# CESR-lab/mgroms

Measured on AMD Instinct MI355X. Metric: V-cycles/sec, seamount 512x512x64 (fine-grid smoother HBM GB/s and % of 8 TB/s: see roofline), higher is better.
Workload: dtype f64; 1 GPU; seamount 512x512x64 (1x1 ranks of 512x512x64), relax_method=FC, ns_pre=3 ns_post=2 ns_coarsest=40, cmatrix=real, interp=linear; levels=6, step=one Vcycle(1), nsmall=8

## Files before the change

### mgroms_amd/csrc/mgx_define.cpp

```cpp
#include "mgx_host.h"

namespace mgx_host {

int dmalloc(double **p, size_t n) {
  void *q = nullptr;
  HIPCHK(hipMalloc(&q, (n ? n : 1) * sizeof(double)));
  HIPCHK(hipMemsetAsync(q, 0, (n ? n : 1) * sizeof(double), S.stream));
  S.allocs.push_back(q);
  *p = (double *)q;
  return 0;
}

int roundup(int a, int m) { return (a + m - 1) / m * m; }

void make_view(LevView &v, int nx, int ny, int nz) {
  v.nx = nx; v.ny = ny; v.nz = nz;
  v.EO = 15;
  v.HO = roundup(16 + ny / 2, 16);
  v.RS = roundup(v.HO + ny / 2 + 1, 16);
  v.plane = (long long)nz * v.RS;
}

int find_grid_levels(int npxg, int npyg, int nx, int ny, int nz, int hold) {
  const int nxg = npxg * nx, nyg = npyg * ny, nzg = nz, ncoarsest = 4, nzmin = 2;
  const int nhoriz = nxg < nyg ? nxg : nyg;
  const int nl1 = 1 + (int)floor(log(nhoriz * 1.0 / ncoarsest * 1.0) / log(2.0));
  if (hold) {
    int l = 1;
    for (int z = nzg; l < nl1 && z != nzmin; l++) z = (z & 1) ? z : z / 2;
    return l;
  }
  const int nl2 = 1 + (int)floor(log(nzg * 1.0 / nzmin * 1.0) / log(2.0));
  return nl1 < nl2 ? nl1 : nl2;
}

void rank_level_table(int rank, std::vector<Level> &T, int npx0, int npy0, int nsmall, int periodic, int hold) {
  const int pi = rank % npx0, pj = rank / npx0;
  int nx = T[0].nx, ny = T[0].ny, nz = T[0].nz, npx = npx0, npy = npy0, incx = 1, incy = 1;
  T[0].npx = npx; T[0].npy = npy; T[0].incx = 1; T[0].incy = 1; T[0].gather = 0; T[0].ngx = 1; T[0].ngy = 1; T[0].key = 0; T[0].color = 0;
  for (int l = 1; l < (int)T.size(); l++) {
    Level &L = T[l];
    if (nz == 1 || (hold && (nz & 1))) { nx /= 2; ny /= 2; } else { nx /= 2; ny /= 2; nz /= 2; }
    L.gather = 0; L.ngx = 1; L.ngy = 1; L.key = 0; L.color = 0;
    if (((nx < ny ? nx : ny) < nsmall) && (npx * npy > 1)) {
      L.gather = 1;
      if (npx > 1) { npx /= 2; nx *= 2; L.ngx = 2; }
      if (npy > 1) { npy /= 2; ny *= 2; L.ngy = 2; }
      incx *= 2; incy *= 2;
    }
    L.nx = nx; L.ny = ny; L.nz = nz; L.npx = npx; L.npy = npy; L.incx = incx; L.incy = incy;
  }
  for (auto &L : T) {
    const int ix = L.incx, iy = L.incy;
    auto col = [&](int s) { const int t = pi + s * ix; return (t >= 0 && t < npx0) ? t : ((periodic & 1) ? ((t % npx0) + npx0) % npx0 : -1); };
    auto row = [&](int s) { const int t = pj + s * iy; return (t >= 0 && t < npy0) ? t : ((periodic & 2) ? ((t % npy0) + npy0) % npy0 : -1); };
    static const int di[8] = {0, 1, 0, -1, -1, 1, 1, -1}, dj[8] = {-1, 0, 1, 0, -1, -1, 1, 1};
    for (int d = 0; d < 8; d++) {
      const int c = col(di[d]), r = row(dj[d]);
      L.neighb[d] = (c >= 0 && r >= 0) ? r * npx0 + c : -1;
    }
  }
  for (int l = 1; l < (int)T.size(); l++) {
    Level &L = T[l];
    if (!L.gather) continue;
    const int ix = L.incx / 2, iy = L.incy / 2;
    const int family = (pi / ix) * ix * iy + npx0 * iy * (pj / iy);
    const int nextfamily = (pi / (2 * ix)) * ix * iy * 4 + npx0 * 2 * iy * (pj / (iy * 2));
    L.color = nextfamily + (pi % ix) + (pj % iy) * ix;
    const int N = ix * npx0;
    L.key = ((family % N) / (ix * iy)) % 2 + 2 * ((family / N) % 2);
  }
}

int gather2d(Level &L, double *src_tmp, double *dst) {
  const int nxc = L.nx / L.ngx, nyc = L.ny / L.ngy, Ng = nxc * nyc;
  rect(src_tmp, L.blk, 3, 1, 1, nyc, 1, nyc, 1, nxc);
  if (!S.ag) return fail("a gather is needed but mgx_set_comm was not called");
  if (S.ag(S.ctx, L.group, L.ngroup, L.blk, L.gbuf, Ng)) return fail("allgather callback failed");
  for (int q = 0; q < L.ngroup; q++) {
    const int l = q % L.ngx, m = q / L.ngx;
    rect(dst, L.gbuf + (size_t)q * Ng, 4, 1, 1, L.ny, 1 + m * nyc, (m + 1) * nyc, 1 + l * nxc, (l + 1) * nxc);
  }
  return 0;
}

void set_window_planes(bool known) {
  for (int l = 0; l < S.nlevs && l < 32; l++) {
    Level &L = S.lev[l];
    if (!L.v.gk || !S.rho_dev || !known) { L.rbs_rho = -1.0; L.rbs_m = 0; L.rbs_rows = L.nz; continue; }
    L.rbs_rho = S.rho_host[l];
    L.rbs_m = mgxk_rbseq_window_planes(L.rbs_rho);
    L.rbs_rows = (L.gdec && !L.gdec_h.empty()) ? mgxk_rbseq_window_rows(L.gdec_h.data(), L.nz) : L.nz;
    if (S.verbose > 1 && S.rank == 0) printf(" level %d: red-black walk contracts by %.4g per plane: %d planes of warm-up%s\n", l + 1, L.rbs_rho, L.rbs_m, L.rbs_m ? "" : " (none: the walk over the whole level stays)");
  }
}

static bool zeta_chain() {
  for (int l = 0; l < S.nlevs; l++) {
    const Level &L = S.lev[l];
    if (L.gather || !all_physical(sides_of(L))) return false;
    if (l > 0 && (2 * L.nx != S.lev[l - 1].nx || 2 * L.ny != S.lev[l - 1].ny)) return false;
  }
  const int D = mgxs_zeta_chain_depth();
  for (int s = 0;; s += D) {
    const int nd = std::min(D, S.nlevs - 1 - s);
    double *a[16];
    for (int d = 0; d <= nd; d++) a[d] = S.lev[s + d].g.zeta;
    mgxs_zeta_chain(S.stream, a, S.lev[s].ny, S.lev[s].nx, nd); S.n_launch++;
    if (s + nd >= S.nlevs - 1) break;
  }
  return true;
}

static int wrap_rmask(Level &L) {
  for (int ax = 0; ax < 2; ax++) {
    if (!(S.periodic & (1 << ax))) continue;
    const int lo = ax == 0 ? 3 : 0, hi = ax == 0 ? 1 : 2;
    const bool first = ax == 0 ? S.pi == 0 : S.pj == 0, last = ax == 0 ? S.pi == S.npx - 1 : S.pj == S.npy - 1;
    const int nn = ax == 0 ? L.nx : L.ny, cnt = (ax == 0 ? L.ny : L.nx) + 2;
    if ((size_t)cnt > S.xbuf_n) return fail("halo buffer too small");
    auto line = [&](double *buf, int op, int c) { if (ax == 0) rect(L.g.rmask, buf, op, 1, 1, L.ny, 0, L.ny + 1, c, c); else rect(L.g.rmask, buf, op, 1, 1, L.ny, c, c, 0, L.nx + 1); };
    int n = 0, peer[2], cn[2], dr[2]; double *sb[2], *rb[2];
    if (first) { line(S.xbuf[lo], 3, 1); peer[n] = L.neighb[lo]; cn[n] = cnt; sb[n] = S.xbuf[lo]; rb[n] = S.xbuf[8 + lo]; dr[n] = lo; n++; }
    if (last) { line(S.xbuf[hi], 3, nn); peer[n] = L.neighb[hi]; cn[n] = cnt; sb[n] = S.xbuf[hi]; rb[n] = S.xbuf[8 + hi]; dr[n] = hi; n++; }
    if (!n) continue;
    CHK(exchange(n, peer, sb, rb, cn, dr));
    if (first) line(S.xbuf[8 + lo], 4, 0);
    if (last) line(S.xbuf[8 + hi], 4, nn + 1);
  }
  return 0;
}

int define_matrices(int what, bool may_return_early) {
  const bool all = what == DM_ALL;
  const bool wait = !(may_return_early && S.async_ops) || (S.rho_dev && S.rb_seq);
  if (S.rho_dev) HIPCHK(hipMemsetAsync(S.rho_dev, 0, sizeof S.rho_host, S.stream));
  const bool chained = !all && zeta_chain();
  if (chained) S.n_zeta_chain++;
  for (int l = 0; l < S.nlevs; l++) {
    Level &L = S.lev[l];
    if (l > 0) {
      Level &F = S.lev[l - 1];
      const int nxc = L.gather ? L.nx / L.ngx : L.nx, nyc = L.gather ? L.ny / L.ngy : L.ny;
      double *src[4] = {F.g.dx, F.g.dy, F.g.zeta, F.g.h};
      double *own[4] = {L.g.dx, L.g.dy, L.g.zeta, L.g.h};
      const double fac[4] = {0.5, 0.5, 0.25, 0.25};
      for (int q = 0; q < 4; q++) {
        if (!all && (q != 2 || chained)) continue;
        mgxs_coarsen2d(S.stream, src[q], L.gather ? L.tmp2[q] : own[q], F.ny, nyc, nxc, fac[q]); S.n_launch++;
        if (L.gather) CHK(gather2d(L, L.tmp2[q], own[q]));
      }
    }
    if (all) CHK(rl_fill_halo(L, L.g.dx, 1, 1, 0));
    if (all) CHK(rl_fill_halo(L, L.g.dy, 1, 1, 0));
    if (!chained) CHK(rl_fill_halo(L, L.g.zeta, 1, 1, 0));
    if (all) CHK(rl_fill_halo(L, L.g.h, 1, 1, 0));
    if (all && l == 0 && S.par.bmask && S.periodic) CHK(wrap_rmask(L));
    mgxs_zr_zw(S.stream, &L.g, S.hlim, S.theta_b, S.theta_s); S.n_launch++;
    CHK(rl_fill_halo(L, L.g.zr, L.nz, 2, 0));
    CHK(rl_fill_halo(L, L.g.zw, L.nz + 1, 2, 0));
    L.g.bmask = S.par.bmask ? 1 : 0;
    if (l > 0 && all) {
      rect(L.g.rmask, 0, 5, 1, 1, L.ny, 0, L.ny + 1, 0, L.nx + 1);
      if (S.par.bmask) {
        if (L.neighb[0] < 0) rect(L.g.rmask, 0, 2, 1, 1, L.ny, 0, 0, 0, L.nx + 1);
        if (L.neighb[1] < 0) rect(L.g.rmask, 0, 2, 1, 1, L.ny, 0, L.ny + 1, L.nx + 1, L.nx + 1);
        if (L.neighb[2] < 0) rect(L.g.rmask, 0, 2, 1, 1, L.ny, L.ny + 1, L.ny + 1, 0, L.nx + 1);
        if (L.neighb[3] < 0) rect(L.g.rmask, 0, 2, 1, 1, L.ny, 0, L.ny + 1, 0, 0);
      }
    }
    L.g.szx = L.g.szy + (size_t)L.nz * (L.ny + 2) * (L.nx + 2);
    mgxs_slopes_ref(S.stream, &L.g); S.n_launch++;
    mgxs_define_matrix(S.stream, &L.g, l == 0, 0); S.n_launch += 2;
    if (S.par.bmask) for (int s = 0; s < 8; s++) CHK(rl_fill_halo(L, L.g.cA + (size_t)s * L.nz * (L.ny + 2) * (L.nx + 2), L.nz, 1, 0, true));
    mgxs_define_matrix(S.stream, &L.g, l == 0, 1); S.n_launch++;
    if (l == 0) {
      mgxm_ref2model(S.stream, L.g.zw, L.g.mzw, L.nz + 1, 2, L.nx, L.ny);
      mgxm_ref2model(S.stream, L.g.dzw, L.g.mdzw, L.nz + 1, 1, L.nx, L.ny);
      mgxm_ref2model(S.stream, L.g.cw, L.g.mcw, L.nz + 1, 1, L.nx, L.ny);
      mgxm_ref2model(S.stream, L.g.zxdy, L.g.mzxdy, L.nz, 1, L.nx, L.ny);
      mgxm_ref2model(S.stream, L.g.zydx, L.g.mzydx, L.nz, 1, L.nx, L.ny);
      S.n_launch += 5;
      if (all) {
        mgxm_ref2model_2d(S.stream, L.g.dx, L.g.mdx, L.nx, L.ny);
        mgxm_ref2model_2d(S.stream, L.g.dy, L.g.mdy, L.nx, L.ny);
        mgxm_ref2model_2d(S.stream, L.g.rmask, L.g.mrmask, L.nx, L.ny);
        S.n_launch += 3;
      }
    }
    if (L.nz <= 1024) { mgxk_convert8(S.stream, &L.v, L.g.cA); S.n_launch++; }
    else for (int s = 0; s < 8; s++) { mgxk_convert(S.stream, &L.v, L.v.cA[s], L.g.cA + (size_t)s * L.nz * (L.ny + 2) * (L.nx + 2), 1, 0, 0); S.n_launch++; }
    mgxs_pivots(S.stream, &L.v); S.n_launch++;
    if (L.v.gk) { mgxk_rbseq_setup(S.stream, &L.v); S.n_launch++; }
    if (L.v.gk && S.rho_dev && l < 32) { mgxk_rbseq_rho(S.stream, &L.v, S.rho_dev + l); S.n_launch++; }
    if (L.v.gk && L.gdec) {
      HIPCHK(hipMemsetAsync(L.gdec, 0, (size_t)L.nz * sizeof(double), S.stream));
      mgxk_rbseq_gdecay(S.stream, &L.v, L.gdec); S.n_launch++;
      if (wait) HIPCHK(hipMemcpyAsync(L.gdec_h.data(), L.gdec, (size_t)L.nz * sizeof(double), hipMemcpyDeviceToHost, S.stream));
    }
    L.v.zy = L.zy_store; L.v.zx = L.zx_store;
    if (L.nz <= 1024) { mgxk_convert2(S.stream, &L.v, L.zy_store, L.zx_store, L.g.szy); S.n_launch++; }
    else { mgxk_convert(S.stream, &L.v, L.zy_store, L.g.szy, 1, 0, 0); mgxk_convert(S.stream, &L.v, L.zx_store, L.g.szx, 1, 0, 0); S.n_launch += 2; }
    L.v.m4 = L.f2d_store[0]; L.v.d4 = L.f2d_store[1]; L.v.m7 = L.f2d_store[2]; L.v.d7 = L.f2d_store[3];
    L.v.h2 = L.f2d_store[4]; L.v.hi2 = L.f2d_store[5]; L.v.ze2 = L.f2d_store[6]; L.v.cffw = L.tab_store[0]; L.v.csw = L.tab_store[1];
    L.v.dx2 = L.zg_store[0]; L.v.dy2 = L.zg_store[1]; L.v.cffr = L.zg_store[2]; L.v.csr = L.zg_store[3];
    if (all) { mgxs_zw_js(S.stream, &L.g, &L.v, S.hlim, S.theta_b, S.theta_s); S.n_launch += 3; }
    else { mgxs_ze2_js(S.stream, &L.g, &L.v); S.n_launch++; }
    if (S.no_mf || S.par.bmask) { L.v.zy = L.v.zx = nullptr; L.v.m4 = nullptr; }
  }
  if (wait) {
    if (S.rho_dev) HIPCHK(hipMemcpyAsync(S.rho_host, S.rho_dev, sizeof S.rho_host, hipMemcpyDeviceToHost, S.stream));
    CHK(sync_stream());
  }
  set_window_planes(wait);
  S.cd_valid = 0;
  S.coef_gen++;
  S.have_matrix = true;
  S.have_geometry = true;
  return 0;
}

ModelView model_view() {
  double *m = S.call_mask ? S.d_rmask_m : (S.par.bmask ? S.lev[0].g.mrmask : nullptr);
  return ModelView{S.d_u, S.d_v, S.d_w, m, S.par.bmask ? 1 : 0};
}

int set_call_mask(const double *rmask, bool dev) {
  S.call_mask = rmask != nullptr;
  if (!rmask) return 0;
  Level &L = S.lev[0];
  const size_t n2 = (size_t)(L.ny + 2) * (L.nx + 2) * sizeof(double);
  HIPCHK(hipMemcpyAsync(S.d_rmask_ref, rmask, n2, dev ? hipMemcpyDeviceToDevice : hipMemcpyHostToDevice, S.stream));
  mgxm_ref2model_2d(S.stream, S.d_rmask_ref, S.d_rmask_m, L.nx, L.ny); S.n_launch++;
  return 0;
}

int flux_halo(Level &L, int face, double *fx) {
  const int lo = face == 0 ? L.neighb[3] : L.neighb[0], hi = face == 0 ? L.neighb[1] : L.neighb[2];
  const int last = face == 0 ? L.nx + 1 : L.ny + 1, cnt = L.nz * (face == 0 ? L.ny : L.nx);
  if (lo < 0) { mgxm_flux_zero_face(S.stream, &L.g, fx, face, 1); S.n_launch++; }
  if (hi < 0) { mgxm_flux_zero_face(S.stream, &L.g, fx, face, last); S.n_launch++; }
  if (lo < 0 && hi < 0) return 0;
  if ((size_t)cnt > S.xbuf_n) return fail("halo buffer too small");
  int n = 0, peer[2], cn[2], dr[2]; double *sb[2], *rb[2];
  if (lo >= 0) { mgxm_flux_face_copy(S.stream, &L.g, fx, S.xbuf[0], face, 1, 0); S.n_launch++; peer[n] = lo; cn[n] = cnt; sb[n] = S.xbuf[0]; rb[n] = S.xbuf[8]; dr[n] = face == 0 ? 3 : 0; n++; }
  if (hi >= 0) { peer[n] = hi; cn[n] = cnt; sb[n] = S.xbuf[2]; rb[n] = S.xbuf[9]; dr[n] = face == 0 ? 1 : 2; n++; }
  if (hi >= 0) HIPCHK(hipMemsetAsync(S.xbuf[2], 0, (size_t)cnt * sizeof(double), S.stream));
  CHK(exchange(n, peer, sb, rb, cn, dr));
  if (hi >= 0) { mgxm_flux_face_copy(S.stream, &L.g, fx, S.xbuf[9], face, last, 1); S.n_launch++; }
  return 0;
}

int compute_rhs_dev() {
  Level &L = S.lev[0];
  TicScope ts(1, "compute_rhs");
  ModelView M = model_view();
  HIPCHK(hipMemsetAsync(L.v.b, 0, L.n3js * sizeof(double), S.stream));
  mgxm_rhs_uf(S.stream, &L.g, &M, S.d_fx); S.n_launch++;
  if (!S.par.bmask) CHK(flux_halo(L, 0, S.d_fx));
  mgxm_rhs_vf(S.stream, &L.g, &M, S.d_fy); S.n_launch++;
  if (!S.par.bmask) CHK(flux_halo(L, 1, S.d_fy));
  mgxm_rhs_wf(S.stream, &L.g, &M, S.d_fz); S.n_launch++;
  mgxm_rhs_accum(S.stream, &L.g, S.d_bm, S.d_fx, S.d_fy, S.d_fz); S.n_launch++;
  mgxm_js_model(S.stream, &L.v, L.v.b, S.d_bm, 1); S.n_launch++;
  return 0;
}

int correct_uvw_dev() {
  Level &L = S.lev[0];
  TicScope ts(1, "correct_uvw");
  ModelView M = model_view();
  mgxm_js_model(S.stream, &L.v, L.v.p, S.d_bm, 0); S.n_launch++;
  mgxm_correct_uvw(S.stream, &L.g, S.d_bm, &M); S.n_launch++;
  return 0;
}

int upload_uvw(const double *u, const double *v, const double *w) {
  Level &L = S.lev[0];
  const size_t nu = (size_t)(L.nx + 1) * (L.ny + 2) * L.nz, nv = (size_t)(L.nx + 2) * (L.ny + 1) * L.nz, nw = (size_t)(L.nx + 2) * (L.ny + 2) * (L.nz + 1);
  HIPCHK(hipMemcpyAsync(S.d_u, u, nu * sizeof(double), hipMemcpyHostToDevice, S.stream));
  HIPCHK(hipMemcpyAsync(S.d_v, v, nv * sizeof(double), hipMemcpyHostToDevice, S.stream));
  HIPCHK(hipMemcpyAsync(S.d_w, w, nw * sizeof(double), hipMemcpyHostToDevice, S.stream));
  return 0;
}

int apply_params(const mgx_params &p) {
  if (streq(p.relax_method, "GS") || streq(p.relax_method, "Gauss-Seidel")) S.method = M_GS;
  else if (streq(p.relax_method, "RB") || streq(p.relax_method, "Red-Black")) S.method = M_RB;
  else if (streq(p.relax_method, "FC") || streq(p.relax_method, "Four-Color")) S.method = M_FC;
  else return fail("unknown relax_method '%s'", p.relax_method);
  S.real = streq(p.cmatrix, "real") ? 1 : 0;
  if (streq(p.interp_type, "linear")) S.linear = 1; else if (streq(p.interp_type, "nearest")) S.linear = 0; else return fail("unknown interp_type '%s'", p.interp_type);
  if (S.linear && streq(p.restrict_type, "linear")) return fail("linear interp + linear restrict is not permitted");
  if (p.aggressive) return fail("aggressive=.true.: coarse2fine_aggressive is not available in the reference either (mg_intergrids.f90:243)");
  S.par = p;
  return 0;
}

}
using namespace mgx_host;

extern "C" {

void mgx_clean(void) {
  if (S.stream || S.inited) (void)hipStreamSynchronize(S.stream);
  p2p_release();
  for (void *q : S.allocs) (void)hipFree(q);
  if (S.h_scalar) (void)hipHostFree(S.h_scalar);
  if (S.kerr) (void)hipHostFree(S.kerr);
  if (S.stream2) { (void)hipStreamSynchronize(S.stream2); (void)hipStreamDestroy(S.stream2); }
  if (S.ev_a) (void)hipEventDestroy(S.ev_a);
  if (S.ev_s) (void)hipEventDestroy(S.ev_s);
  if (S.ev_x) (void)hipEventDestroy(S.ev_x);
  tt_collect();
  hipStream_t st = S.stream; const int vb = S.verbose; const std::vector<int> opts = options_carried();
  mgx_exchange_fn ex = S.ex; mgx_allreduce_fn ar = S.ar; mgx_allgather_fn ag = S.ag; void *ctx = S.ctx; const bool nat = S.native_rccl;
  std::vector<std::string> tn = S.tt_names; std::vector<HostTic> th = S.tt_host; const int tnb = S.tt_nblev;
  static thread_local double tsave[32][32]; static thread_local long long csave[32][32];
  memcpy(tsave, S.tt_time, sizeof tsave); memcpy(csave, S.tt_calls, sizeof csave);
  S = State();
  S.tt_names = tn; S.tt_host = th; S.tt_nblev = tnb; memcpy(S.tt_time, tsave, sizeof tsave); memcpy(S.tt_calls, csave, sizeof csave);
  S.native_rccl = nat;
  S.stream = st; S.verbose = vb; options_restore(opts); S.ex = ex; S.ar = ar; S.ag = ag; S.ctx = ctx;
}

int mgx_init(int nx, int ny, int nz, int npx, int npy, int rank, const mgx_params *par) {
  if (S.inited) mgx_clean();
  int ndev = 0;
  if (hipGetDeviceCount(&ndev) != hipSuccess || ndev == 0) return fail("no HIP device visible: libmgx has no CPU path");
  mgx_params p;
  if (par) p = *par; else { mgx_params_default(&p); CHK(mgx_read_namelist(nullptr, &p)); }
  CHK(apply_params(p));
  if (nx < 2 || ny < 2 || nz < 2 || (nx & 1) || (ny & 1) || (nz & 1)) return fail("nx,ny,nz must be even and >= 2 (got %d %d %d)", nx, ny, nz);
  if (npx < 1 || npy < 1 || (npx & (npx - 1)) || (npy & (npy - 1))) return fail("the process grid must be powers of two in both directions (got %d x %d)", npx, npy);
  if (rank < 0 || rank >= npx * npy) return fail("rank %d outside the %d x %d process grid", rank, npx, npy);
  if (S.periodic && npx * npy > 1 && !S.ex)
    return fail("option \"periodic\" = %d needs a single rank (process grid %d x %d) or connected ranks: install the hooks (mgx_set_comm, mgx_rccl_connect) before mgx_init", S.periodic, npx, npy);
  S.npx = npx; S.npy = npy; S.nranks = npx * npy; S.rank = rank; S.pi = rank % npx; S.pj = rank / npx;
  S.nlevs = find_grid_levels(npx, npy, nx, ny, nz, S.hold_odd_nz);
  if (S.nlevs < 1) return fail("grid %dx%dx%d too small for a multigrid hierarchy", nx * npx, ny * npy, nz);
  S.lev.assign(S.nlevs, Level());
  S.lev[0].nx = nx; S.lev[0].ny = ny; S.lev[0].nz = nz;
  rank_level_table(rank, S.lev, npx, npy, S.par.nsmall, S.periodic, S.hold_odd_nz);
  for (int l = 0; l < S.nlevs; l++) {
    const Level &L = S.lev[l];
    if ((L.nx & 1) || (L.ny & 1) || L.nz < 2) return fail("level %d has local size %dx%dx%d: odd sizes are not supported (assumptions:1-2)", l + 1, L.nx, L.ny, L.nz);
  }
  for (int l = 1; l < S.nlevs; l++) {
    Level &L = S.lev[l];
    if (!L.gather) continue;
    std::vector<std::pair<int, int>> mem;
    for (int r = 0; r < S.nranks; r++) {
      std::vector<Level> T(S.nlevs);
      T[0].nx = nx; T[0].ny = ny; T[0].nz = nz;
      rank_level_table(r, T, npx, npy, S.par.nsmall, 0, S.hold_odd_nz);
      if (T[l].color == L.color) mem.push_back({T[l].key, r});
    }
    std::sort(mem.begin(), mem.end());
    L.ngroup = (int)mem.size();
    if (L.ngroup != L.ngx * L.ngy) return fail("gather group of level %d has %d members, expected %d", l + 1, L.ngroup, L.ngx * L.ngy);
    for (int q = 0; q < L.ngroup; q++) L.group[q] = mem[q].second;
  }
  size_t max_part = 1;
  for (int l = 0; l < S.nlevs; l++) {
    Level &L = S.lev[l];
    make_view(L.v, L.nx, L.ny, L.nz);
    L.n3js = (size_t)(L.nx + 2) * L.v.plane;
    CHK(dmalloc(&L.v.p, L.n3js)); CHK(dmalloc(&L.v.b, L.n3js)); CHK(dmalloc(&L.v.r, L.n3js));
    for (int s = 0; s < 8; s++) CHK(dmalloc(&L.v.cA[s], L.n3js));
    CHK(dmalloc(&L.v.bet, L.n3js)); CHK(dmalloc(&L.v.gam, L.n3js));
    CHK(dmalloc(&L.v.p1, (size_t)(L.nx + 2) * L.v.RS)); CHK(dmalloc(&L.p1b, (size_t)(L.nx + 2) * L.v.RS)); L.v.p1w = nullptr;
    { double *q = nullptr; CHK(dmalloc(&q, (size_t)(L.nx + 2) / 2 + 1)); L.ksp_done = (unsigned int *)q; L.ksp_seq = 0; }
    CHK(dmalloc(&L.zy_store, L.n3js)); CHK(dmalloc(&L.zx_store, L.n3js));
    L.v.zy = L.v.zx = nullptr;
    for (int q = 0; q < 7; q++) CHK(dmalloc(&L.f2d_store[q], (size_t)(L.nx + 2) * L.v.RS));
    for (int q = 0; q < 2; q++) CHK(dmalloc(&L.tab_store[q], (size_t)L.nz + 1));
    L.v.m4 = L.v.d4 = L.v.m7 = L.v.d7 = L.v.h2 = L.v.hi2 = L.v.ze2 = nullptr; L.v.cffw = L.v.csw = nullptr;
    for (int q = 0; q < 2; q++) CHK(dmalloc(&L.zg_store[q], (size_t)(L.nx + 2) * L.v.RS));
    for (int q = 2; q < 4; q++) CHK(dmalloc(&L.zg_store[q], (size_t)L.nz + 1));
    L.v.dx2 = L.v.dy2 = nullptr; L.v.cffr = L.v.csr = nullptr;
    L.v.gk = L.v.ag58 = L.v.u1 = nullptr; L.v.d0w = nullptr;
    if (S.method == M_RB && S.real) {
      CHK(dmalloc(&L.v.gk, L.n3js));
      CHK(dmalloc(&L.gdec, (size_t)L.nz)); L.gdec_h.assign((size_t)L.nz, 0.0);
      CHK(dmalloc(&L.v.ag58, (size_t)2 * (L.nx + 2) * L.v.RS)); CHK(dmalloc(&L.v.u1, (size_t)(L.nx + 2) * L.v.RS));
      { double *q = nullptr; CHK(dmalloc(&q, (size_t)(L.nx / 8 + 2) * 8 + 16)); L.rbs_flag = (unsigned int *)q; L.rbs_seq = 0; }
    }
    const size_t n2 = (size_t)(L.ny + 2) * (L.nx + 2);
    L.g.nx = L.nx; L.g.ny = L.ny; L.g.nz = L.nz;
    CHK(dmalloc(&L.g.dx, n2)); CHK(dmalloc(&L.g.dy, n2)); CHK(dmalloc(&L.g.zeta, n2)); CHK(dmalloc(&L.g.h, n2));
    CHK(dmalloc(&L.g.rmask, n2)); L.g.bmask = 0;
    CHK(dmalloc(&L.g.zr, (size_t)(L.ny + 4) * (L.nx + 4) * L.nz));
    CHK(dmalloc(&L.g.zw, (size_t)(L.ny + 4) * (L.nx + 4) * (L.nz + 1)));
    CHK(dmalloc(&L.g.cw, n2 * (L.nz + 1)));
    L.g.dzw = L.g.zxdy = L.g.zydx = nullptr;
    L.g.mzw = L.g.mdzw = L.g.mzxdy = L.g.mzydx = L.g.mcw = L.g.mdx = L.g.mdy = L.g.mrmask = nullptr;
    if (l == 0) {
      CHK(dmalloc(&L.g.dzw, n2 * (L.nz + 1))); CHK(dmalloc(&L.g.zxdy, n2 * L.nz)); CHK(dmalloc(&L.g.zydx, n2 * L.nz));
      CHK(dmalloc(&L.g.mzw, n2 * (L.nz + 1))); CHK(dmalloc(&L.g.mdzw, n2 * (L.nz + 1))); CHK(dmalloc(&L.g.mcw, n2 * (L.nz + 1)));
      CHK(dmalloc(&L.g.mzxdy, n2 * L.nz)); CHK(dmalloc(&L.g.mzydx, n2 * L.nz));
      CHK(dmalloc(&L.g.mdx, n2)); CHK(dmalloc(&L.g.mdy, n2)); CHK(dmalloc(&L.g.mrmask, n2));
    }
    if (L.gather) {
      const int nxc = L.nx / L.ngx, nyc = L.ny / L.ngy;
      L.vs = L.v;
      make_view(L.vs, nxc, nyc, L.nz);
      const size_t ns = (size_t)(nxc + 2) * L.vs.plane;
      CHK(dmalloc(&L.vs.b, ns)); CHK(dmalloc(&L.vs.p, ns));
      const size_t Ng = (size_t)L.nz * (nyc + 2) * (nxc + 2);
      CHK(dmalloc(&L.blk, Ng)); CHK(dmalloc(&L.gbuf, Ng * L.ngroup));
      for (int q = 0; q < 4; q++) CHK(dmalloc(&L.tmp2[q], (size_t)(nyc + 2) * (nxc + 2)));
    }
    size_t np = (size_t)mgxk_residual_nblocks(&L.v);
    if (l == 1) { const size_t nf = (size_t)mgxk_residual_restrict_grid(&S.lev[0].v, &L.v); if (nf > np) np = nf; }
    if (np > max_part) max_part = np;
  }
  S.npartial = (int)max_part;
  CHK(dmalloc(&S.d_partial, max_part));
  CHK(dmalloc(&S.d_scalar, 8));
  if (S.method == M_RB && S.real) CHK(dmalloc(&S.rho_dev, 32));
  HIPCHK(hipHostMalloc((void **)&S.h_scalar, 8 * sizeof(double)));
  HIPCHK(hipHostMalloc((void **)&S.kerr, 64, hipHostMallocMapped));
  *S.kerr = 0;
  if (S.nranks > 1) {
    HIPCHK(hipStreamCreateWithFlags(&S.stream2, hipStreamNonBlocking));
    HIPCHK(hipEventCreateWithFlags(&S.ev_a, hipEventDisableTiming)); HIPCHK(hipEventCreateWithFlags(&S.ev_s, hipEventDisableTiming)); HIPCHK(hipEventCreateWithFlags(&S.ev_x, hipEventDisableTiming));
  }
  Level &L1 = S.lev[0];
  S.ref_scratch_n = (size_t)8 * L1.nz * (L1.ny + 2) * (L1.nx + 2);
  CHK(dmalloc(&S.ref_scratch, S.ref_scratch_n));
  CHK(dmalloc(&S.slope_scratch, S.ref_scratch_n / 4));
  for (auto &L : S.lev) { L.g.cA = S.ref_scratch; L.g.szy = S.slope_scratch; L.g.szx = nullptr; }
  S.xbuf_n = (size_t)(L1.nz + 1) * 2 * ((L1.nx > L1.ny ? L1.nx : L1.ny) + 4);
  if (S.par.bmask && S.nranks > 1) {
    const size_t n4 = (size_t)8 * L1.nz * (L1.nx > L1.ny ? L1.nx : L1.ny);
    if (n4 > S.xbuf_n) S.xbuf_n = n4;
  }
  for (int q = 0; q < 16; q++) CHK(dmalloc(&S.xbuf[q], S.xbuf_n));
  CHK(dmalloc(&S.d_u, (size_t)(L1.nx + 1) * (L1.ny + 2) * L1.nz));
  CHK(dmalloc(&S.d_v, (size_t)(L1.nx + 2) * (L1.ny + 1) * L1.nz));
  CHK(dmalloc(&S.d_w, (size_t)(L1.nx + 2) * (L1.ny + 2) * (L1.nz + 1)));
  CHK(dmalloc(&S.d_fx, (size_t)(L1.nx + 2) * (L1.ny + 2) * (L1.nz + 1)));
  CHK(dmalloc(&S.d_fy, (size_t)(L1.nx + 2) * (L1.ny + 2) * (L1.nz + 1)));
  CHK(dmalloc(&S.d_fz, (size_t)(L1.nx + 2) * (L1.ny + 2) * (L1.nz + 1)));
  CHK(dmalloc(&S.d_bm, (size_t)(L1.nx + 2) * (L1.ny + 2) * L1.nz));
  CHK(dmalloc(&S.d_rmask_ref, (size_t)(L1.nx + 2) * (L1.ny + 2))); CHK(dmalloc(&S.d_rmask_m, (size_t)(L1.nx + 2) * (L1.ny + 2)));
  S.call_mask = false;
  CHK(sync_stream());
  S.use_small = getenv("MGX_NO_SMALL") ? 0 : 1;
  S.no_mf = getenv("MGX_NO_MF") ? 1 : 0;
  options_from_env();
  if (getenv("MGX_P2P_TIMEOUT_MS")) (void)mgxk_set_p2p_timeout(atof(getenv("MGX_P2P_TIMEOUT_MS")));
  S.inited = true;
  if (S.verbose && S.rank == 0) {
    printf(" Non hydrostatic parameters:\n   - solver_prec   : %g\n   - solver_maxiter: %d\n   - nsmall        : %d\n   - ns_coarsest   : %d\n"
           "   - ns_pre        : %d\n   - ns_post       : %d\n   - cmatrix       : %s\n   - relax_method  : %s\n   - interp_type   : %s\n"
           "   - restrict_type : %s\n   - aggressive    : %c\n   - netcdf_output : %c\n   - bmask         : %c\n\n",
           p.solver_prec, p.solver_maxiter, p.nsmall, p.ns_coarsest, p.ns_pre, p.ns_post, p.cmatrix, p.relax_method, p.interp_type,
           p.restrict_type, p.aggressive ? 'T' : 'F', p.netcdf_output ? 'T' : 'F', p.bmask ? 'T' : 'F');
    printf(" - print grid information:\n");
    for (int l = 0; l < S.nlevs; l++) {
      const Level &L = S.lev[l];
      printf("  lev=%2d: %3d x%3d x%3d on %3d x%3d procs%s\n", l + 1, L.nx, L.ny, L.nz, L.npx, L.npy, L.gather ? " / gather" : "");
    }
  }
  return 0;
}

}
```

### mgroms_amd/csrc/mgx_device.h

```cpp
#pragma once
#include "mgx_internal.h"

#define WAVE 64
#define NT_LOAD(ptr) __builtin_nontemporal_load(ptr)
#define NT2_STORE(v, ptr) __builtin_nontemporal_store(v, ptr)
template <bool NT> __device__ __forceinline__ double ld_stream(const double *p) { return NT ? NT_LOAD(p) : *p; }
__device__ __forceinline__ void st_rt(double *p, double v, int nt) { if (nt) __builtin_nontemporal_store(v, p); else *p = v; }
__device__ __forceinline__ double ld_rt(const double *p, int nt) { return nt ? __builtin_nontemporal_load(p) : *p; }
static inline int level_streams(const LevView *L) { return (double)L->nx * L->ny * L->nz * 72.0 > 256e6; }

#define COL_POS(L, jh, jodd, c, jm, jp)                                 \
  {                                                                     \
    if (jodd) { c = L.HO + jh; jm = L.EO + jh; jp = jm + 1; }           \
    else      { c = L.EO + jh + 1; jm = L.HO + jh; jp = jm + 1; }       \
  }

#define COL_IMAGES(L, i, j, ph)                                                                                              \
  const bool mS = ph.S && j == 1, mN = ph.N && j == L.ny, mW = ph.W && i == 1, mE = ph.E && i == L.nx;                       \
  const int cS = L.EO, cN = jpos(L, L.ny + 1);                                                                               \
  const long long oW = 0, oE = (long long)(L.nx + 1) * L.plane;
#define COL_STORE(ST, p, o, ro, c, v)                                                                                        \
  {                                                                                                                          \
    if (ST) NT2_STORE(v, p + o + ro + c); else p[o + ro + c] = v;                                                            \
    if (mS) p[o + ro + cS] = v;                                                                                              \
    if (mN) p[o + ro + cN] = v;                                                                                              \
    if (mW) { p[oW + ro + c] = v; if (mS) p[oW + ro + cS] = v; if (mN) p[oW + ro + cN] = v; }                                \
    if (mE) { p[oE + ro + c] = v; if (mS) p[oE + ro + cS] = v; if (mN) p[oE + ro + cN] = v; }                                \
  }
#define SNAP_MIRROR(idx) { w1[idx] = v1; r1[idx] = v1; }
#define COL_SNAPSHOT(L, RS, i, c, v)                                                                                          \
  {                                                                                                                          \
    double *w1 = L.p1w, *r1 = L.p1;                                                                                          \
    const long long so = (long long)i * RS, sW = 0, sE = (long long)(L.nx + 1) * RS;                                  \
    const double v1 = v;                                                                                                     \
    w1[so + c] = v1;                                                                                                         \
    if (mS) SNAP_MIRROR(so + cS)                                                                                             \
    if (mN) SNAP_MIRROR(so + cN)                                                                                             \
    if (mW) { SNAP_MIRROR(sW + c) if (mS) SNAP_MIRROR(sW + cS) if (mN) SNAP_MIRROR(sW + cN) }                                \
    if (mE) { SNAP_MIRROR(sE + c) if (mS) SNAP_MIRROR(sE + cS) if (mN) SNAP_MIRROR(sE + cN) }                                \
  }

__device__ __forceinline__ void mirror_store(const LevView &L, double *__restrict__ a, const long long ro, const int j, const int i,
                                             const int c, const double v, const Sides ph) {
  const bool mS = ph.S && j == 1, mN = ph.N && j == L.ny, mW = ph.W && i == 1, mE = ph.E && i == L.nx;
  if (!(mS | mN | mW | mE)) return;
  const int cS = L.EO, cN = jpos(L, L.ny + 1);
  const long long o = (long long)i * L.plane + ro, oW = ro, oE = (long long)(L.nx + 1) * L.plane + ro;
  if (mS) a[o + cS] = v;
  if (mN) a[o + cN] = v;
  if (mW) { a[oW + c] = v; if (mS) a[oW + cS] = v; if (mN) a[oW + cN] = v; }
  if (mE) { a[oE + c] = v; if (mS) a[oE + cS] = v; if (mN) a[oE + cN] = v; }
}

extern thread_local hipError_t mgx_pending_error;
static inline void mgx_before_launch() { const hipError_t e = hipGetLastError(); if (e != hipSuccess && mgx_pending_error == hipSuccess) mgx_pending_error = e; }
static inline int mgx_launched() { return hipGetLastError() == hipSuccess ? 1 : 0; }

static inline dim3 col_grid(int ncol_half, int nplanes, int z = 1) { return dim3((ncol_half + WAVE - 1) / WAVE, (nplanes + 3) / 4, z); }

#define RCP_REF(b) ({ const double b_ = (b); double r_ = __builtin_amdgcn_rcp(b_); double e_ = __builtin_fma(-b_, r_, 1.0); r_ = __builtin_fma(r_, e_, r_); \
                      e_ = __builtin_fma(-b_, r_, 1.0); __builtin_fma(r_, e_, r_); })
#define DIVC(a, b, rb) ({ const double a_ = (a); const double q_ = a_ * (rb); const double e_ = __builtin_fma(-(b), q_, a_); __builtin_fma(e_, (rb), q_); })
#define LD_PAIR(ptr, A, B) { double2 t2_; __builtin_memcpy(&t2_, (ptr), 16); A = t2_.x; B = t2_.y; }

__device__ __forceinline__ double wave_shr1(double x) {
  int lo = __double2loint(x), hi = __double2hiint(x);
  lo = __builtin_amdgcn_update_dpp(0, lo, 0x138, 0xf, 0xf, false);
  hi = __builtin_amdgcn_update_dpp(0, hi, 0x138, 0xf, 0xf, false);
  return __hiloint2double(hi, lo);
}
__device__ __forceinline__ double wave_shl1(double x) {
  int lo = __double2loint(x), hi = __double2hiint(x);
  lo = __builtin_amdgcn_update_dpp(0, lo, 0x130, 0xf, 0xf, false);
  hi = __builtin_amdgcn_update_dpp(0, hi, 0x130, 0xf, 0xf, false);
  return __hiloint2double(hi, lo);
}
```

### mgroms_amd/csrc/mgx_kernels.hip

```cpp
#include "mgx_switches.h"
#include "mgx_operator.h"

#define RES_RHS(ko) b[ko]
#define RES_SINK(ro, ko, rr) { r[ko] = rr; mirror_store(L, r, ro, jcol, i, c, rr, ph); acc = acc + rr * rr; }
template <bool REAL>
__global__ __launch_bounds__(256) void k_residual(LevView L, double *__restrict__ partial, int want_norm, int gx, int gy, Sides ph, int stream) {
  int bx, by, bz;
  op_block_map(gx, gy, bx, by, bz);
  const int jh = bx * WAVE + threadIdx.x;
  const int i = 1 + by * blockDim.y + threadIdx.y;
  const int jodd = bz == 0;
  double acc = 0.0;
  if (jh < (L.ny >> 1) && i <= L.nx) {
    int c, jm, jp;
    COL_POS(L, jh, jodd, c, jm, jp)
    const double *__restrict__ b = L.b;
    double *__restrict__ r = L.r;
    OP_COLUMN(OP_P, RES_RHS, RES_SINK)
  }
  if (!want_norm) return;
  OP_BLOCK_SUM(acc, partial, blockIdx.x)
}

#define RES_RHS_MF(ko) ld_rt(b + ko, stream)
#define RES_SINK_MF(ro, ko, rr) { st_rt(r + ko, rr, stream); mirror_store(L, r, ro, jodd ? 2 * jh + 1 : 2 * jh + 2, i, c, rr, ph); acc = acc + rr * rr; }
template <bool REAL>
__global__ __launch_bounds__(256) void k_residual_mf(LevView L, double *__restrict__ partial, int want_norm, int gx, int gy, Sides ph, int stream) {
  int bx, by, bz;
  op_block_map(gx, gy, bx, by, bz);
  const int jh = bx * WAVE + threadIdx.x;
  const int i = 1 + by * blockDim.y + threadIdx.y;
  const int jodd = bz == 0;
  double acc = 0.0;
  if (jh < (L.ny >> 1) && i <= L.nx) {
    int c, jm, jp;
    COL_POS(L, jh, jodd, c, jm, jp)
    const double *__restrict__ b = L.b;
    double *__restrict__ r = L.r;
    OP_COLUMN_MF(OP_P, OP_P2, RES_RHS_MF, RES_SINK_MF)
  }
  if (!want_norm) return;
  OP_BLOCK_SUM(acc, partial, blockIdx.x)
}

__global__ __launch_bounds__(256) void k_sumsq(LevView L, const double *__restrict__ a, double *__restrict__ partial) {
  const int jh = blockIdx.x * WAVE + threadIdx.x;
  const int i = 1 + blockIdx.y * blockDim.y + threadIdx.y;
  double acc = 0.0;
  if (jh < (L.ny >> 1) && i <= L.nx) {
    const int c = blockIdx.z == 0 ? L.HO + jh : L.EO + jh + 1;
    const long long o = (long long)i * L.plane + c;
    for (int k = 0; k < L.nz; k++) { const double v = a[o + (long long)k * L.RS]; acc += v * v; }
  }
  OP_BLOCK_SUM(acc, partial, (blockIdx.z * gridDim.y + blockIdx.y) * gridDim.x + blockIdx.x)
}

__global__ __launch_bounds__(256) void k_dot(LevView L, const double *__restrict__ a, const double *__restrict__ b, double *__restrict__ partial) {
  const int jh = blockIdx.x * WAVE + threadIdx.x;
  const int i = 1 + blockIdx.y * blockDim.y + threadIdx.y;
  double acc = 0.0;
  if (jh < (L.ny >> 1) && i <= L.nx) {
    const int c = blockIdx.z == 0 ? L.HO + jh : L.EO + jh + 1;
    const long long o = (long long)i * L.plane + c;
    for (int k = 0; k < L.nz; k++) acc += a[o + (long long)k * L.RS] * b[o + (long long)k * L.RS];
  }
  OP_BLOCK_SUM(acc, partial, (blockIdx.z * gridDim.y + blockIdx.y) * gridDim.x + blockIdx.x)
}

__global__ __launch_bounds__(256) void k_reduce_partials(const double *__restrict__ partial, int n, double *__restrict__ out) {
  __shared__ double red[256];
  double s = 0.0;
  for (int q = threadIdx.x; q < n; q += 256) s += partial[q];
  red[threadIdx.x] = s;
  __syncthreads();
  for (int off = 128; off > 0; off >>= 1) {
    if ((int)threadIdx.x < off) red[threadIdx.x] += red[threadIdx.x + off];
    __syncthreads();
  }
  if (threadIdx.x == 0) out[0] = red[0];
}

struct LevChain { LevView v[5]; };
template <int DEP>
__global__ __launch_bounds__(256) void k_restrict_chain(LevChain Ch, Sides ph) {
  constexpr int E = 1 << DEP;
  __shared__ double buf[E * E * E + (E / 2) * (E / 2) * (E / 2)];
  double *cur = buf, *nxt = buf + E * E * E;
  const LevView &F = Ch.v[0];
  const int nbj = F.ny / E, nbk = F.nz / E;
  int bb = blockIdx.x;
  const int kb = bb % nbk; bb /= nbk;
  const int jb = bb % nbj, ib = bb / nbj;
  for (int t = threadIdx.x; t < E * E * E; t += 256) {
    const int hj = t % (E / 2), par = (t / (E / 2)) & 1, kk = (t / E) % E, ii = t / (E * E);
    const int jj = 2 * hj + par;
    const int i = ib * E + ii + 1, j = jb * E + jj + 1, k = kb * E + kk + 1;
    cur[(ii * E + kk) * E + jj] = F.r[(long long)i * F.plane + (long long)(k - 1) * F.RS + jpos(F, j)];
  }
  __syncthreads();
#pragma unroll
  for (int d = 1; d <= DEP; d++) {
    const int e = E >> (d - 1), h = e >> 1;
    const LevView &C = Ch.v[d];
    for (int t = threadIdx.x; t < h * h * h; t += 256) {
      const int jc = t % h, kc = (t / h) % h, ic = t / (h * h);
      const int iA = 2 * ic, iB = iA + 1, k0 = 2 * kc, k1 = k0 + 1, jA = 2 * jc, jB = jA + 1;
#define CH(ii_, kk_, jj_) cur[((ii_) * e + (kk_)) * e + (jj_)]
      const double z = CH(iA, k0, jA) + CH(iB, k0, jA) + CH(iA, k0, jB) + CH(iB, k0, jB) + CH(iA, k1, jA) + CH(iB, k1, jA) + CH(iA, k1, jB) + CH(iB, k1, jB);
#undef CH
      nxt[(ic * h + kc) * h + jc] = z;
      const int i2 = ib * h + ic + 1, j2 = jb * h + jc + 1, k2 = kb * h + kc + 1, cj = jpos(C, j2);
      const long long rc = (long long)(k2 - 1) * C.RS, oc = (long long)i2 * C.plane + rc + cj;
      C.b[oc] = z; mirror_store(C, C.b, rc, j2, i2, cj, z, ph);
      C.r[oc] = z; mirror_store(C, C.r, rc, j2, i2, cj, z, ph);
      C.p[oc] = 0.0; mirror_store(C, C.p, rc, j2, i2, cj, 0.0, ph);
    }
    __syncthreads();
    double *sw = cur; cur = nxt; nxt = sw;
  }
}

__global__ __launch_bounds__(256) void k_fine2coarse(LevView F, LevView C, double *__restrict__ dst, Sides ph, int stream, double *__restrict__ dup, double *__restrict__ zero, int KC) {
  const int j2 = 1 + blockIdx.x * WAVE + threadIdx.x;
  const int i2 = 1 + blockIdx.y * blockDim.y + threadIdx.y;
  if (j2 > C.ny || i2 > C.nx) return;
  const int ka = 1 + blockIdx.z * KC, kb = ka + KC - 1 < C.nz ? ka + KC - 1 : C.nz;
  const int i = 2 * i2 - 1;
  const int po = F.HO + (j2 - 1), pe = F.EO + j2;
  const double *__restrict__ x = F.r;
  const long long o0 = (long long)i * F.plane, o1 = o0 + F.plane;
  const long long oc = (long long)i2 * C.plane + jpos(C, j2);
  for (int k2 = ka; k2 <= kb; k2++) {
    const long long r0 = (long long)(2 * k2 - 2) * F.RS, r1 = r0 + F.RS;
    const double z = ld_rt(x + o0 + r0 + po, stream) + ld_rt(x + o1 + r0 + po, stream) + ld_rt(x + o0 + r0 + pe, stream) + ld_rt(x + o1 + r0 + pe, stream)
                   + ld_rt(x + o0 + r1 + po, stream) + ld_rt(x + o1 + r1 + po, stream) + ld_rt(x + o0 + r1 + pe, stream) + ld_rt(x + o1 + r1 + pe, stream);
    dst[oc + (long long)(k2 - 1) * C.RS] = z;
    mirror_store(C, dst, (long long)(k2 - 1) * C.RS, j2, i2, jpos(C, j2), z, ph);
    if (dup) { dup[oc + (long long)(k2 - 1) * C.RS] = z; mirror_store(C, dup, (long long)(k2 - 1) * C.RS, j2, i2, jpos(C, j2), z, ph); }
    if (zero) { zero[oc + (long long)(k2 - 1) * C.RS] = 0.0; mirror_store(C, zero, (long long)(k2 - 1) * C.RS, j2, i2, jpos(C, j2), 0.0, ph); }
  }
}

template <bool WR>
__global__ __launch_bounds__(256) void k_coarse2fine_nearest(LevView F, LevView C, const double *__restrict__ xc, Sides ph, int stream) {
  const int j2 = 1 + blockIdx.x * WAVE + threadIdx.x;
  const int k2 = 1 + blockIdx.y * blockDim.y + threadIdx.y;
  const int i2 = 1 + blockIdx.z;
  if (j2 > C.ny || k2 > C.nz) return;
  const int i = 2 * i2 - 1;
  const int po = F.HO + (j2 - 1), pe = F.EO + j2;
  const long long o0 = (long long)i * F.plane, o1 = o0 + F.plane;
  double *__restrict__ rf = F.r;
  double *__restrict__ pf = F.p;
#define PUT(k, OO, PP, val) { const long long ro_ = (long long)((k)-1) * F.RS, t_ = OO + ro_ + PP; const double v_ = (val), w_ = ld_rt(pf + t_, stream) + v_; if (WR) st_rt(rf + t_, v_, stream); st_rt(pf + t_, w_, stream); \
    const int jf_ = (PP == po) ? 2 * j2 - 1 : 2 * j2, if_ = (OO == o0) ? i : i + 1; \
    if (WR) mirror_store(F, rf, ro_, jf_, if_, PP, v_, ph); mirror_store(F, pf, ro_, jf_, if_, PP, w_, ph); }
  const double v = xc[(long long)i2 * C.plane + (long long)(k2 - 1) * C.RS + jpos(C, j2)];
  const int k = 2 * k2 - 1;
  PUT(k, o0, po, v); PUT(k + 1, o0, po, v); PUT(k, o0, pe, v); PUT(k + 1, o0, pe, v);
  PUT(k, o1, po, v); PUT(k + 1, o1, po, v); PUT(k, o1, pe, v); PUT(k + 1, o1, pe, v);
#undef PUT
}

template <bool WR, bool SK>
__global__ __launch_bounds__(256) void k_coarse2fine_run(LevView F, LevView C, const double *__restrict__ xc, Sides ph, int stream, int KC) {
  const int lane = threadIdx.x;
  const int j2 = 1 + blockIdx.x * WAVE + lane;
  const int i2 = 1 + blockIdx.z;
  const int nz = C.nz;
  const int ka = 1 + (blockIdx.y * blockDim.y + threadIdx.y) * KC;
  if (ka > nz) return;
  const int kb = ka + KC - 1 < nz ? ka + KC - 1 : nz;
  const bool live = j2 <= C.ny;
  const int jl = live ? j2 : C.ny + 1;
  const int i = 2 * i2 - 1;
  const int po = F.HO + (j2 - 1), pe = F.EO + j2;
  const int c0 = jpos(C, jl), cm = jpos(C, jl - 1), cp = jpos(C, jl + 1 <= C.ny + 1 ? jl + 1 : jl);
  const long long q0 = (long long)i2 * C.plane, qm = q0 - C.plane, qp = q0 + C.plane;
  const long long o0 = (long long)i * F.plane, o1 = o0 + F.plane;
  double *__restrict__ rf = F.r;
  double *__restrict__ pf = F.p;
#define ROW(kk, v)                                                                                                  \
  {                                                                                                                 \
    const long long ro_ = (long long)(((kk) < 1 ? 1 : ((kk) > nz ? nz : (kk))) - 1) * C.RS;                          \
    const double t0_ = xc[qm + ro_ + c0], t1_ = xc[q0 + ro_ + c0], t2_ = xc[qp + ro_ + c0];                         \
    v[1] = t0_; v[4] = t1_; v[7] = t2_;                                                                             \
    v[0] = __shfl_up(t0_, 1, WAVE); v[3] = __shfl_up(t1_, 1, WAVE); v[6] = __shfl_up(t2_, 1, WAVE);                 \
    v[2] = __shfl_down(t0_, 1, WAVE); v[5] = __shfl_down(t1_, 1, WAVE); v[8] = __shfl_down(t2_, 1, WAVE);           \
     \
                                                          \
    const double e0_ = xc[qm + ro_ + ce], e1_ = xc[q0 + ro_ + ce], e2_ = xc[qp + ro_ + ce];                         \
    if (lane == 0) { v[0] = e0_; v[3] = e1_; v[6] = e2_; }                                                          \
    if (lane == WAVE - 1) { v[2] = e0_; v[5] = e1_; v[8] = e2_; }                                                   \
  }
#define LOADP(kk, v)                                                                                                \
  {                                                                                                                 \
    const int kq_ = (kk) <= kb ? (kk) : kb;                                                                         \
    _Pragma("unroll") for (int h_ = 0; h_ < 2; h_++) {                                                              \
      const long long ro_ = (long long)(2 * kq_ - 2 + h_) * F.RS;                                                   \
      if (!SK) v[4 * h_ + 0] = ld_rt(pf + o0 + ro_ + pol, stream);                                                  \
      v[4 * h_ + 1] = ld_rt(pf + o0 + ro_ + pel, stream);                                                           \
      v[4 * h_ + 2] = ld_rt(pf + o1 + ro_ + pol, stream); v[4 * h_ + 3] = ld_rt(pf + o1 + ro_ + pel, stream);       \
    }                                                                                                               \
  }
#define LOADP0(kk, v)                                                                                               \
  if (SK && edge0 && live) {                                                                                        \
    const int kq_ = (kk) <= kb ? (kk) : kb;                                                                         \
    _Pragma("unroll") for (int h_ = 0; h_ < 2; h_++) v[4 * h_ + 0] = ld_rt(pf + o0 + (long long)(2 * kq_ - 2 + h_) * F.RS + po, stream); \
  }
#define PUT(k, Q, val) if (!(SK && (Q) == 0) || edge0) { const long long OO_ = ((Q) & 2) ? o1 : o0; const int PP_ = ((Q) & 1) ? pe : po;                      \
    const long long ro_ = (long long)((k)-1) * F.RS, t_ = OO_ + ro_ + PP_; const double v_ = (val), w_ = pc[4 * half + (Q)] + v_;                     \
    if (WR) st_rt(rf + t_, v_, stream); st_rt(pf + t_, w_, stream);                                                                                    \
    const int jf_ = ((Q) & 1) ? 2 * j2 : 2 * j2 - 1, if_ = ((Q) & 2) ? i + 1 : i;                                                                      \
    if (WR) mirror_store(F, rf, ro_, jf_, if_, PP_, v_, ph); mirror_store(F, pf, ro_, jf_, if_, PP_, w_, ph); }
  const bool edge0 = (ph.S && j2 == 1) || (ph.W && i2 == 1);
  const int ce = lane == 0 ? cm : (lane == WAVE - 1 ? cp : c0);
  const int pol = live ? po : F.HO + (C.ny - 1), pel = live ? pe : F.EO + C.ny;
  const double a = 9. / 16., b = 3. / 16., c = 1. / 16., d = 27. / 64., e = 9. / 64., f = 3. / 64., g = 1. / 64.;
  double pc[8], pa[8], pb[8];
  double lo[9], x[9], hi[9], nw[9];
#pragma unroll
  for (int q = 0; q < 9; q++) lo[q] = hi[q] = nw[q] = 0.0;
#pragma unroll
  for (int q = 0; q < 8; q++) pa[q] = pb[q] = 0.0;
  LOADP(ka, pa) LOADP0(ka, pa)
  ROW(ka - 1, lo)
  ROW(ka, x)
  ROW(ka + 1, hi)
#define STEP(kk, CUR, NXT)                                                                                          \
  {                                                                                                                 \
    const int k2 = (kk);                                                                                            \
    LOADP(k2 + 1, NXT) LOADP0(k2 + 1, NXT)                                                                          \
    ROW(k2 + 2, nw)                                                                                                 \
    _Pragma("unroll") for (int q = 0; q < 8; q++) pc[q] = CUR[q];                                                   \
    if (live) {                                                                                                     \
      const double xmm = x[0], x0m = x[1], xpm = x[2], xm0 = x[3], x00 = x[4], xp0 = x[5], xmp = x[6], x0p = x[7], xpp = x[8]; \
      _Pragma("unroll") for (int half = 0; half < 2; half++) {                                                      \
        const int k = 2 * k2 - 1 + half;                                                            \
        if (k == 1) {                                        \
          PUT(1, 0, +a * x00 + c * xmm + b * xm0 + b * x0m);                                                   \
          PUT(1, 1, +a * x00 + c * xpm + b * xp0 + b * x0m);                                                   \
          PUT(1, 2, +a * x00 + c * xmp + b * xm0 + b * x0p);                                                   \
          PUT(1, 3, +a * x00 + c * xpp + b * xp0 + b * x0p);                                                   \
        } else if (k == 2 * nz) {                                            \
          PUT(k, 0, 0.5 * (a * x00 + c * xmm + b * xm0 + b * x0m));                                            \
          PUT(k, 1, 0.5 * (a * x00 + c * xpm + b * xp0 + b * x0m));                                            \
          PUT(k, 2, 0.5 * (a * x00 + c * xmp + b * xm0 + b * x0p));                                            \
          PUT(k, 3, 0.5 * (a * x00 + c * xpp + b * xp0 + b * x0p));                                            \
        } else {                            \
          const double *__restrict__ y = half ? hi : lo;                                                            \
          const double ymm = y[0], y0m = y[1], ypm = y[2], ym0 = y[3], y00 = y[4], yp0 = y[5], ymp = y[6], y0p = y[7], ypp = y[8]; \
          PUT(k, 0, +d * x00 + f * xmm + e * xm0 + e * x0m + e * y00 + g * ymm + f * ym0 + f * y0m);           \
          PUT(k, 1, +d * x00 + f * xpm + e * xp0 + e * x0m + e * y00 + g * ypm + f * yp0 + f * y0m);           \
          PUT(k, 2, +d * x00 + f * xmp + e * xm0 + e * x0p + e * y00 + g * ymp + f * ym0 + f * y0p);           \
          PUT(k, 3, +d * x00 + f * xpp + e * xp0 + e * x0p + e * y00 + g * ypp + f * yp0 + f * y0p);           \
        }                                                                                                           \
      }                                                                                                             \
    }                                                                                                               \
    _Pragma("unroll") for (int q = 0; q < 9; q++) { lo[q] = x[q]; x[q] = hi[q]; hi[q] = nw[q]; }                    \
  }
  int kk = ka;
  for (; kk + 1 <= kb; kk += 2) {
    STEP(kk, pa, pb)
    STEP(kk + 1, pb, pa)
  }
  if (kk <= kb) STEP(kk, pa, pb)
#undef STEP
#undef ROW
#undef PUT
#undef LOADP
#undef LOADP0
}

__global__ __launch_bounds__(256) void k_halo_phys(LevView L, double *__restrict__ a, Sides ph) {
  const int q = blockIdx.x * blockDim.x + threadIdx.x;
  const long long ro = (long long)blockIdx.y * L.RS;
  const int nx = L.nx, ny = L.ny;
  if (q < nx) {
    const long long o = (long long)(q + 1) * L.plane + ro;
    if (ph.S) a[o + jpos(L, 0)] = a[o + jpos(L, 1)];
    if (ph.N) a[o + jpos(L, ny + 1)] = a[o + jpos(L, ny)];
  } else if (q < nx + ny) {
    const int j = q - nx + 1, c = jpos(L, j);
    if (ph.W) a[ro + c] = a[L.plane + ro + c];
    if (ph.E) a[(long long)(nx + 1) * L.plane + ro + c] = a[(long long)nx * L.plane + ro + c];
  } else if (q == nx + ny) {
    const long long oE = (long long)(nx + 1) * L.plane + ro, oI = (long long)nx * L.plane + ro;
    if (ph.S && ph.W) a[ro + jpos(L, 0)] = a[L.plane + ro + jpos(L, 1)];
    if (ph.S && ph.E) a[oE + jpos(L, 0)] = a[oI + jpos(L, 1)];
    if (ph.N && ph.E) a[oE + jpos(L, ny + 1)] = a[oI + jpos(L, ny)];
    if (ph.N && ph.W) a[ro + jpos(L, ny + 1)] = a[L.plane + ro + jpos(L, ny)];
  }
}

typedef double v2d __attribute__((ext_vector_type(2)));
template <bool NT>
__global__ __launch_bounds__(256) void k_halo_wrap(LevView L, double *__restrict__ a, int im, int jm) {
  const int nx = L.nx, ny = L.ny;
  const long long t = (long long)blockIdx.x * blockDim.x + threadIdx.x;
  const int c0 = jpos(L, 0), cN = jpos(L, ny + 1);
  const int s0 = jm == 1 ? jpos(L, ny) : jpos(L, 1), sN = jm == 1 ? jpos(L, 1) : jpos(L, ny);
  if (blockIdx.y < 2) {
    if (!im || 2 * t >= L.plane) return;
    const int east = blockIdx.y;
    const int src = im == 1 ? (east ? 1 : nx) : (east ? nx : 1), dst = east ? nx + 1 : 0;
    const double *__restrict__ s = a + (long long)src * L.plane;
    const long long e = 2 * t;
    v2d v = NT ? __builtin_nontemporal_load((const v2d *)(s + e)) : *(const v2d *)(s + e);
    if (jm) {
      const int c = (int)(e % L.RS);
      const long long ro = e - c;
      if (c == c0) v.x = s[ro + s0]; else if (c + 1 == c0) v.y = s[ro + s0];
      if (c == cN) v.x = s[ro + sN]; else if (c + 1 == cN) v.y = s[ro + sN];
    }
    v2d *d = (v2d *)(a + (long long)dst * L.plane + e);
    if (NT) __builtin_nontemporal_store(v, d); else *d = v;
  } else {
    if (!jm) return;
    const int i0 = im ? 1 : 0, np = im ? nx : nx + 2;
    if (t >= (long long)np * L.nz) return;
    const long long o = (long long)(i0 + (int)(t / L.nz)) * L.plane + (t % L.nz) * L.RS;
    a[o + c0] = a[o + s0];
    a[o + cN] = a[o + sN];
  }
}

__global__ void k_halo_mixed_corners(LevView L, double *__restrict__ a, int mSW, int mSE, int mNE, int mNW) {
  const int k = blockIdx.x * blockDim.x + threadIdx.x;
  if (k >= L.nz) return;
  const long long ro = (long long)k * L.RS;
  const int nx = L.nx, ny = L.ny;
  const long long W0 = ro, W1 = L.plane + ro, E0 = (long long)(nx + 1) * L.plane + ro, E1 = (long long)nx * L.plane + ro;
  const int j0 = jpos(L, 0), j1 = jpos(L, 1), jn = jpos(L, ny), jn1 = jpos(L, ny + 1);
  if (mSW == 1) a[W0 + j0] = a[W1 + j0]; else if (mSW == 2) a[W0 + j0] = a[W0 + j1];
  if (mSE == 1) a[E0 + j0] = a[E1 + j0]; else if (mSE == 2) a[E0 + j0] = a[E0 + j1];
  if (mNE == 1) a[E0 + jn1] = a[E1 + jn1]; else if (mNE == 2) a[E0 + jn1] = a[E0 + jn];
  if (mNW == 1) a[W0 + jn1] = a[W1 + jn1]; else if (mNW == 2) a[W0 + jn1] = a[W0 + jn];
}

struct HaloBufs { double *b[8]; int present[8]; };
__device__ __forceinline__ bool halo_elem(const LevView &L, int dir, int q, int k, int unpack, long long &e, long long &t) {
  const int nx = L.nx, ny = L.ny;
  int i, j, n;
  switch (dir) {
    case 0: n = nx; i = q + 1; j = unpack ? 0 : 1; break;
    case 1: n = ny; j = q + 1; i = unpack ? nx + 1 : nx; break;
    case 2: n = nx; i = q + 1; j = unpack ? ny + 1 : ny; break;
    case 3: n = ny; j = q + 1; i = unpack ? 0 : 1; break;
    case 4: n = 1; i = unpack ? 0 : 1; j = unpack ? 0 : 1; break;
    case 5: n = 1; i = unpack ? nx + 1 : nx; j = unpack ? 0 : 1; break;
    case 6: n = 1; i = unpack ? nx + 1 : nx; j = unpack ? ny + 1 : ny; break;
    default: n = 1; i = unpack ? 0 : 1; j = unpack ? ny + 1 : ny; break;
  }
  if (q >= n) return false;
  e = (long long)i * L.plane + (long long)k * L.RS + jpos(L, j);
  t = (long long)k * n + q;
  return true;
}
__device__ __forceinline__ int halo_opp(int d) { return d < 4 ? (d ^ 2) : 4 + ((d - 4) ^ 2); }
template <bool MIXED>
__global__ void k_halo_pack_all(LevView L, double *__restrict__ a, HaloBufs hb, int unpack) {
  const int dir = blockIdx.z, pr = hb.present[dir];
  if (MIXED ? (pr != HALO_PEER && !(pr == HALO_SELF && unpack)) : !pr) return;
  const int q = blockIdx.x * blockDim.x + threadIdx.x;
  long long e, t;
  if (!halo_elem(L, dir, q, blockIdx.y, unpack, e, t)) return;
  if (MIXED && pr == HALO_SELF) {
    long long es, ts;
    halo_elem(L, halo_opp(dir), q, blockIdx.y, 0, es, ts);
    a[e] = a[es];
    return;
  }
  double *__restrict__ buf = hb.b[dir];
  if (unpack) a[e] = buf[t]; else buf[t] = a[e];
}

__device__ long long g_p2p_timeout_ticks = 500000000LL;
struct HaloP2P {
  int drop;
  unsigned long long *flag[8];
  unsigned long long seq;
  unsigned int *counter;
  int *err;
  int mSW, mSE, mNE, mNW;
  int blk0[9];
  int ipt;
  int nreal;
};
__device__ __forceinline__ int halo_dir(const HaloP2P &pp) {
  int dir = 0;
#pragma unroll
  for (int d = 1; d < 8; d++) if ((int)blockIdx.x >= pp.blk0[d]) dir = d;
  return dir;
}
__device__ __forceinline__ bool halo_item(const LevView &L, const HaloP2P &pp, int dir, int r, int unpack, int &q, int &k, long long &e, long long &t) {
  const int n = (dir == 0 || dir == 2) ? L.nx : ((dir == 1 || dir == 3) ? L.ny : 1);
  const int w = (((int)blockIdx.x - pp.blk0[dir]) * pp.ipt + r) * blockDim.x + threadIdx.x;
  if (w >= n * L.nz) return false;
  k = w / n; q = w - k * n;
  return halo_elem(L, dir, q, k, unpack, e, t);
}
struct HaloXchg { double *rbuf[8]; double *lbuf[8]; unsigned long long *rflag[8]; unsigned long long *lflag[8]; int present[8]; };
__device__ __forceinline__ void halo_store(const LevView &L, const HaloP2P &pp, double *__restrict__ a, int dir, int q, int k, long long e, double v) {
  const int nx = L.nx, ny = L.ny;
  a[e] = v;
  const long long ro = (long long)k * L.RS, W0 = ro, E0 = (long long)(nx + 1) * L.plane + ro;
  if (dir == 0) { if (q == 0 && pp.mSW == 1) a[W0 + jpos(L, 0)] = v; if (q == nx - 1 && pp.mSE == 1) a[E0 + jpos(L, 0)] = v; }
  else if (dir == 2) { if (q == 0 && pp.mNW == 1) a[W0 + jpos(L, ny + 1)] = v; if (q == nx - 1 && pp.mNE == 1) a[E0 + jpos(L, ny + 1)] = v; }
  else if (dir == 3) { if (q == 0 && pp.mSW == 2) a[W0 + jpos(L, 0)] = v; if (q == ny - 1 && pp.mNW == 2) a[W0 + jpos(L, ny + 1)] = v; }
  else if (dir == 1) { if (q == 0 && pp.mSE == 2) a[E0 + jpos(L, 0)] = v; if (q == ny - 1 && pp.mNE == 2) a[E0 + jpos(L, ny + 1)] = v; }
}
template <bool MIXED>
__global__ __launch_bounds__(256) void k_halo_exchange(LevView L, double *__restrict__ a, HaloXchg hx, HaloP2P pp) {
  const int dir = halo_dir(pp);
  int q, k; long long e, t;
  if (MIXED && hx.present[dir] != HALO_PEER) {
    const int sdir = hx.present[dir] == HALO_SELF ? halo_opp(dir) : dir;
    for (int r = 0; r < pp.ipt; r++) {
      if (!halo_item(L, pp, dir, r, 1, q, k, e, t)) continue;
      long long es, ts;
      halo_elem(L, sdir, q, k, 0, es, ts);
      halo_store(L, pp, a, dir, q, k, e, a[es]);
    }
    return;
  }
  for (int r = 0; r < pp.ipt; r++)
    if (halo_item(L, pp, dir, r, 0, q, k, e, t)) hx.rbuf[dir][t] = a[e];
  asm volatile("s_waitcnt vmcnt(0)" ::: "memory");
  __syncthreads();
  __shared__ int ok;
  if (threadIdx.x == 0) {
    __builtin_amdgcn_fence(__ATOMIC_RELEASE, "");
    asm volatile("s_waitcnt vmcnt(0)" ::: "memory");
    if (__hip_atomic_fetch_add(pp.counter, 1u, __ATOMIC_ACQ_REL, __HIP_MEMORY_SCOPE_AGENT) == (MIXED ? (unsigned int)pp.nreal : gridDim.x) - 1) {
      __hip_atomic_store(pp.counter, 0u, __ATOMIC_RELAXED, __HIP_MEMORY_SCOPE_AGENT);
      __threadfence_system();
      for (int d = 0; d < 8; d++)
        if ((MIXED ? hx.present[d] == HALO_PEER : hx.present[d] != 0) && !pp.drop) __hip_atomic_store(hx.rflag[d], pp.seq, __ATOMIC_RELEASE, __HIP_MEMORY_SCOPE_SYSTEM);
    }
    ok = 0;
    const long long t0 = wall_clock64(), tmax = g_p2p_timeout_ticks;
    while (true) {
      if (__hip_atomic_load(hx.lflag[dir], __ATOMIC_ACQUIRE, __HIP_MEMORY_SCOPE_SYSTEM) >= pp.seq) { ok = 1; break; }
      if (wall_clock64() - t0 > tmax) break;
      __builtin_amdgcn_s_sleep(4);
    }
  }
  __syncthreads();
  if (!ok) { if (threadIdx.x == 0) *pp.err = 1; return; }
  __threadfence_system();
  for (int r = 0; r < pp.ipt; r++) {
    if (!halo_item(L, pp, dir, r, 1, q, k, e, t)) continue;
    halo_store(L, pp, a, dir, q, k, e, __builtin_nontemporal_load(hx.lbuf[dir] + t));
  }
}

__global__ void k_convert(LevView L, double *__restrict__ js, double *__restrict__ ref, int nslot, int slot, int dir) {
  const long long n = (long long)L.nz * (L.ny + 2) * (L.nx + 2);
  const long long t = (long long)blockIdx.x * blockDim.x + threadIdx.x;
  if (t >= n) return;
  const int k = (int)(t % L.nz);
  const long long ji = t / L.nz;
  const int j = (int)(ji % (L.ny + 2)), i = (int)(ji / (L.ny + 2));
  const long long e = (long long)i * L.plane + (long long)k * L.RS + jpos(L, j);
  if (dir == 0) js[e] = ref[t * nslot + slot]; else ref[t * nslot + slot] = js[e];
}

struct Slots8 { double *s[8]; };
__global__ __launch_bounds__(256) void k_convert_slots(LevView L, Slots8 out, const double *__restrict__ ref, int TJ) {
  extern __shared__ double lds[];
  const int nz = L.nz, cs = nz + 1, H = (TJ >> 1) * cs;
  const int i = blockIdx.y, j0 = blockIdx.x * TJ, sl = blockIdx.z;
  const int nj = min(TJ, L.ny + 2 - j0);
  const long long n3 = (long long)nz * (L.ny + 2) * (L.nx + 2);
  const double *__restrict__ src = ref + (long long)sl * n3 + ((long long)i * (L.ny + 2) + j0) * nz;
  const int run = nj * nz;
  const bool p2 = (nz & (nz - 1)) == 0;
  const int lz = 31 - __builtin_clz(nz);
  constexpr int U = 8;
  const int nt = blockDim.x;
  for (int r0 = threadIdx.x; r0 < run; r0 += U * nt) {
    double v[U];
#pragma unroll
    for (int u = 0; u < U; u++) { const int r = r0 + u * nt; v[u] = r < run ? src[r] : 0.0; }
#pragma unroll
    for (int u = 0; u < U; u++) {
      const int r = r0 + u * nt;
      if (r < run) { const int jl = p2 ? (r >> lz) : r / nz, k = r - jl * nz; lds[(jl & 1) * H + (jl >> 1) * cs + k] = v[u]; }
    }
  }
  __syncthreads();
  double *__restrict__ os = out.s[sl] + (long long)i * L.plane;
  const int hj = TJ >> 1;
  for (int t = threadIdx.x; t < TJ * nz; t += nt) {
    const int q = t % hj, par = (t / hj) & 1, k = t / TJ;
    const int jl = 2 * q + par;
    if (jl < nj) os[(long long)k * L.RS + (par ? L.HO : L.EO) + ((j0 + jl) >> 1)] = lds[par * H + q * cs + k];
  }
}

__global__ void k_gather_place(LevView C, double *__restrict__ dstjs, const double *__restrict__ blk, int nxc, int nyc, int l, int m) {
  const long long n = (long long)C.nz * nyc * nxc;
  const long long t = (long long)blockIdx.x * blockDim.x + threadIdx.x;
  if (t >= n) return;
  const int k = (int)(t % C.nz);
  const long long ji = t / C.nz;
  const int j = 1 + (int)(ji % nyc), i = 1 + (int)(ji / nyc);
  const double v = blk[((long long)i * (nyc + 2) + j) * C.nz + k];
  dstjs[(long long)(i + l * nxc) * C.plane + (long long)k * C.RS + jpos(C, j + m * nyc)] = v;
}
__global__ void k_block_to_ref(LevView Cs, const double *__restrict__ js, double *__restrict__ blk) {
  const long long n = (long long)Cs.nz * (Cs.ny + 2) * (Cs.nx + 2);
  const long long t = (long long)blockIdx.x * blockDim.x + threadIdx.x;
  if (t >= n) return;
  const int k = (int)(t % Cs.nz);
  const long long ji = t / Cs.nz;
  const int j = (int)(ji % (Cs.ny + 2)), i = (int)(ji / (Cs.ny + 2));
  blk[t] = js[(long long)i * Cs.plane + (long long)k * Cs.RS + jpos(Cs, j)];
}
struct GatherP2P { double *dst[4]; unsigned long long *flag[4]; int ng, me; unsigned long long seq; unsigned int *counter; int *err; };
__global__ void k_gather_push(LevView Cs, const double *__restrict__ js, GatherP2P gp) {
  const long long n = (long long)Cs.nz * (Cs.ny + 2) * (Cs.nx + 2);
  for (long long t = (long long)blockIdx.x * blockDim.x + threadIdx.x; t < n; t += (long long)gridDim.x * blockDim.x) {
    const int j = (int)(t % (Cs.ny + 2));
    const long long ik = t / (Cs.ny + 2);
    const int k = (int)(ik % Cs.nz), i = (int)(ik / Cs.nz);
    const double v = js[(long long)i * Cs.plane + (long long)k * Cs.RS + jpos(Cs, j)];
    for (int q = 0; q < gp.ng; q++) gp.dst[q][t] = v;
  }
  asm volatile("s_waitcnt vmcnt(0)" ::: "memory");
  __syncthreads();
  if (threadIdx.x == 0) {
    __builtin_amdgcn_fence(__ATOMIC_RELEASE, "");
    asm volatile("s_waitcnt vmcnt(0)" ::: "memory");
    if (__hip_atomic_fetch_add(gp.counter, 1u, __ATOMIC_ACQ_REL, __HIP_MEMORY_SCOPE_AGENT) == gridDim.x - 1) {
      __hip_atomic_store(gp.counter, 0u, __ATOMIC_RELAXED, __HIP_MEMORY_SCOPE_AGENT);
      __threadfence_system();
      for (int q = 0; q < gp.ng; q++)
        if (q != gp.me) __hip_atomic_store(gp.flag[q], gp.seq, __ATOMIC_RELEASE, __HIP_MEMORY_SCOPE_SYSTEM);
    }
  }
}
__global__ void k_gather_place_wait(LevView C, double *__restrict__ dstjs, const double *__restrict__ blk, int nxc, int nyc, int l, int m,
                                    unsigned long long *flag, unsigned long long seq, int *err) {
  if (flag) {
    __shared__ int ok;
    if (threadIdx.x == 0) {
      ok = 0;
      const long long t0 = wall_clock64(), tmax = g_p2p_timeout_ticks;
      while (true) {
        if (__hip_atomic_load(flag, __ATOMIC_ACQUIRE, __HIP_MEMORY_SCOPE_SYSTEM) >= seq) { ok = 1; break; }
        if (wall_clock64() - t0 > tmax) break;
        __builtin_amdgcn_s_sleep(4);
      }
    }
    __syncthreads();
    if (!ok) { if (threadIdx.x == 0) *err = 1; return; }
    __threadfence_system();
  }
  const long long n = (long long)C.nz * nyc * nxc;
  for (long long t = (long long)blockIdx.x * blockDim.x + threadIdx.x; t < n; t += (long long)gridDim.x * blockDim.x) {
    const int j = 1 + (int)(t % nyc);
    const long long ik = t / nyc;
    const int k = (int)(ik % C.nz), i = 1 + (int)(ik / C.nz);
    const double v = __builtin_nontemporal_load(blk + ((long long)i * C.nz + k) * (nyc + 2) + j);
    dstjs[(long long)(i + l * nxc) * C.plane + (long long)k * C.RS + jpos(C, j + m * nyc)] = v;
  }
}
__global__ void k_split(LevView C, LevView Cs, const double *__restrict__ pc, double *__restrict__ dst, int l, int m) {
  const long long n = (long long)Cs.nz * (Cs.ny + 2) * (Cs.nx + 2);
  const long long t = (long long)blockIdx.x * blockDim.x + threadIdx.x;
  if (t >= n) return;
  const int k = (int)(t % Cs.nz);
  const long long ji = t / Cs.nz;
  const int j = (int)(ji % (Cs.ny + 2)), i = (int)(ji / (Cs.ny + 2));
  dst[(long long)i * Cs.plane + (long long)k * Cs.RS + jpos(Cs, j)] =
      pc[(long long)(i + l * Cs.nx) * C.plane + (long long)k * C.RS + jpos(C, j + m * Cs.ny)];
}


__global__ void k_divc_selftest(const double *__restrict__ a, const double *__restrict__ b, int n, unsigned long long *bad) {
  const int t = blockIdx.x * blockDim.x + threadIdx.x;
  if (t >= n) return;
  const double q = a[t] / b[t], rb = RCP_REF(b[t]), c = DIVC(a[t], b[t], rb);
  if (__double_as_longlong(q) != __double_as_longlong(c)) atomicAdd(bad, 1ull);
}

extern "C" {

int mgxk_residual_nblocks(const LevView *L) { dim3 g = col_grid(L->ny / 2, L->nx, 2); return g.x * g.y * g.z; }
void mgxk_residual(hipStream_t st, const LevView *L, double *partial, double *out, int real, int want_norm, Sides ph) {
  dim3 blk(WAVE, 4), g3 = col_grid(L->ny / 2, L->nx, 2), grd(g3.x * g3.y * 2);
  const int gx = g3.x, gy = g3.y;
  if (L->zy != nullptr && L->nz >= 3) {
    if (real) hipLaunchKernelGGL((k_residual_mf<true>), grd, blk, 0, st, *L, partial, want_norm, gx, gy, ph, level_streams(L));
    else hipLaunchKernelGGL((k_residual_mf<false>), grd, blk, 0, st, *L, partial, want_norm, gx, gy, ph, level_streams(L));
  } else if (real) hipLaunchKernelGGL((k_residual<true>), grd, blk, 0, st, *L, partial, want_norm, gx, gy, ph, level_streams(L));
  else hipLaunchKernelGGL((k_residual<false>), grd, blk, 0, st, *L, partial, want_norm, gx, gy, ph, level_streams(L));
  if (want_norm) hipLaunchKernelGGL(k_reduce_partials, dim3(1), dim3(256), 0, st, partial, (int)grd.x, out);
}
void mgxk_reduce(hipStream_t st, const double *partial, int n, double *out) { hipLaunchKernelGGL(k_reduce_partials, dim3(1), dim3(256), 0, st, partial, n, out); }
void mgxk_sumsq(hipStream_t st, const LevView *L, const double *a, double *partial, double *out) {
  dim3 blk(WAVE, 4), grd = col_grid(L->ny / 2, L->nx, 2);
  hipLaunchKernelGGL(k_sumsq, grd, blk, 0, st, *L, a, partial);
  hipLaunchKernelGGL(k_reduce_partials, dim3(1), dim3(256), 0, st, partial, (int)(grd.x * grd.y * grd.z), out);
}
void mgxk_dot(hipStream_t st, const LevView *L, const double *a, const double *b, double *partial, double *out) {
  dim3 blk(WAVE, 4), grd = col_grid(L->ny / 2, L->nx, 2);
  hipLaunchKernelGGL(k_dot, grd, blk, 0, st, *L, a, b, partial);
  hipLaunchKernelGGL(k_reduce_partials, dim3(1), dim3(256), 0, st, partial, (int)(grd.x * grd.y * grd.z), out);
}
void mgxk_restrict_chain(hipStream_t st, const LevView *const *levels, int dep, Sides ph) {
  LevChain Ch;
  for (int q = 0; q <= dep && q < 5; q++) Ch.v[q] = *levels[q];
  for (int q = dep + 1; q < 5; q++) Ch.v[q] = *levels[dep];
  const LevView &F = Ch.v[0];
  const int E = 1 << dep;
  const dim3 grd((unsigned)((F.nx / E) * (F.ny / E) * (F.nz / E)));
  switch (dep) {
    case 1: hipLaunchKernelGGL(k_restrict_chain<1>, grd, dim3(256), 0, st, Ch, ph); break;
    case 2: hipLaunchKernelGGL(k_restrict_chain<2>, grd, dim3(256), 0, st, Ch, ph); break;
    case 3: hipLaunchKernelGGL(k_restrict_chain<3>, grd, dim3(256), 0, st, Ch, ph); break;
    default: hipLaunchKernelGGL(k_restrict_chain<4>, grd, dim3(256), 0, st, Ch, ph); break;
  }
}
void mgxk_fine2coarse(hipStream_t st, const LevView *F, const LevView *C, double *dst, Sides ph, double *dup, double *zero) {
  dim3 grd = col_grid(C->ny, C->nx);
  const long long waves = (long long)grd.x * grd.y * 4;
  long long nchunk = (8192 + waves - 1) / waves;
  if (nchunk > C->nz) nchunk = C->nz;
  if (nchunk < 1) nchunk = 1;
  const int KC = (int)((C->nz + nchunk - 1) / nchunk);
  grd.z = (C->nz + KC - 1) / KC;
  hipLaunchKernelGGL(k_fine2coarse, grd, dim3(WAVE, 4), 0, st, *F, *C, dst, ph, level_streams(F), dup, zero, KC);
}
void mgxk_coarse2fine(hipStream_t st, const LevView *F, const LevView *C, const double *src, int linear, Sides ph, int keep_r, int skip1) {
  if (linear) {
    int KC = mgx_switches().c2f_kc > 0 ? mgx_switches().c2f_kc : 16;
    const long long wav = (long long)((C->ny + WAVE - 1) / WAVE) * C->nx;
    while (KC > 1 && wav * ((C->nz + KC - 1) / KC) < 2048) KC >>= 1;
    if (KC > C->nz) KC = C->nz;
    const int nrun = (C->nz + KC - 1) / KC, byr = nrun >= 4 ? 4 : nrun;
    dim3 blk(WAVE, byr), grd((C->ny + WAVE - 1) / WAVE, (nrun + byr - 1) / byr, C->nx);
    const int nt = mgx_switches().c2f_nt >= 0 ? mgx_switches().c2f_nt : level_streams(F);
    if (keep_r) hipLaunchKernelGGL((k_coarse2fine_run<true, false>), grd, blk, 0, st, *F, *C, src, ph, nt, KC);
    else if (skip1 && !(F->nx & 1) && !(F->ny & 1)) hipLaunchKernelGGL((k_coarse2fine_run<false, true>), grd, blk, 0, st, *F, *C, src, ph, nt, KC);
    else hipLaunchKernelGGL((k_coarse2fine_run<false, false>), grd, blk, 0, st, *F, *C, src, ph, nt, KC);
    return;
  }
  const int by = C->nz >= 4 ? 4 : C->nz;
  dim3 blk(WAVE, by), grd((C->ny + WAVE - 1) / WAVE, (C->nz + by - 1) / by, C->nx);
  if (keep_r) hipLaunchKernelGGL((k_coarse2fine_nearest<true>), grd, blk, 0, st, *F, *C, src, ph, level_streams(F));
  else hipLaunchKernelGGL((k_coarse2fine_nearest<false>), grd, blk, 0, st, *F, *C, src, ph, level_streams(F));
}
void mgxk_divc_selftest(hipStream_t st, const double *a, const double *b, int n, unsigned long long *bad) {
  hipLaunchKernelGGL(k_divc_selftest, dim3((n + 255) / 256), dim3(256), 0, st, a, b, n, bad);
}
void mgxk_halo_phys(hipStream_t st, const LevView *L, double *a, Sides ph) {
  const int n = L->nx + L->ny + 1;
  hipLaunchKernelGGL(k_halo_phys, dim3((n + 255) / 256, L->nz), dim3(256), 0, st, *L, a, ph);
}
void mgxk_halo_wrap(hipStream_t st, const LevView *L, double *a, int im, int jm) {
  if (!im && !jm) return;
  const long long npl = im ? (L->plane / 2 + 255) / 256 : 0, nj = jm ? ((long long)(L->nx + 2) * L->nz + 255) / 256 : 0;
  const dim3 grd((unsigned)(npl > nj ? npl : nj), 3), blk(256);
  if (level_streams(L)) hipLaunchKernelGGL((k_halo_wrap<true>), grd, blk, 0, st, *L, a, im, jm);
  else hipLaunchKernelGGL((k_halo_wrap<false>), grd, blk, 0, st, *L, a, im, jm);
}
void mgxk_halo_mixed_corners(hipStream_t st, const LevView *L, double *a, int mSW, int mSE, int mNE, int mNW) {
  hipLaunchKernelGGL(k_halo_mixed_corners, dim3((L->nz + 63) / 64), dim3(64), 0, st, *L, a, mSW, mSE, mNE, mNW);
}
void mgxk_halo_pack_all(hipStream_t st, const LevView *L, double *a, double *const *bufs, const int *present, int unpack) {
  HaloBufs hb;
  for (int d = 0; d < 8; d++) { hb.b[d] = bufs[d]; hb.present[d] = present[d]; }
  const int n = L->nx > L->ny ? L->nx : L->ny;
  bool mixed = false;
  for (int d = 0; d < 8; d++) mixed |= present[d] > HALO_PEER;
  if (mixed) hipLaunchKernelGGL((k_halo_pack_all<true>), dim3((n + 63) / 64, L->nz, 8), dim3(64), 0, st, *L, a, hb, unpack);
  else hipLaunchKernelGGL((k_halo_pack_all<false>), dim3((n + 63) / 64, L->nz, 8), dim3(64), 0, st, *L, a, hb, unpack);
}
void mgxk_halo_p2p(hipStream_t st, const LevView *L, double *a, double *const *rbuf, double *const *lbuf, unsigned long long *const *rflag,
                   unsigned long long *const *lflag, const int *present, unsigned long long seq, unsigned int *counter, int *err, const int *mixed, int drop) {
  HaloXchg hx; HaloP2P pp;
  pp.drop = drop;
  const int maxblk = mgx_switches().p2p_maxblk;
  long long items = 0;
  for (int d = 0; d < 8; d++) if (present[d] == HALO_PEER) items += (long long)L->nz * ((d == 0 || d == 2) ? L->nx : ((d == 1 || d == 3) ? L->ny : 1));
  pp.ipt = (int)((items + 256LL * maxblk - 1) / (256LL * maxblk)) + 1;
  const int ipt_min = mgx_switches().p2p_ipt;
  if (pp.ipt < ipt_min) pp.ipt = ipt_min;
  const int per = 256 * pp.ipt;
  int nb = 0;
  pp.nreal = 0;
  for (int d = 0; d < 8; d++) {
    hx.rbuf[d] = rbuf[d]; hx.lbuf[d] = lbuf[d]; hx.rflag[d] = rflag[d]; hx.lflag[d] = lflag[d]; hx.present[d] = present[d];
    pp.flag[d] = nullptr;
    pp.blk0[d] = nb;
    const int nd = present[d] ? (L->nz * ((d == 0 || d == 2) ? L->nx : ((d == 1 || d == 3) ? L->ny : 1)) + per - 1) / per : 0;
    nb += nd;
    if (present[d] == HALO_PEER) pp.nreal += nd;
  }
  pp.blk0[8] = nb;
  for (int d = 7; d >= 0; d--) if (!present[d]) pp.blk0[d] = nb + 1;
  pp.seq = seq; pp.counter = counter; pp.err = err;
  pp.mSW = mixed[0]; pp.mSE = mixed[1]; pp.mNE = mixed[2]; pp.mNW = mixed[3];
  if (nb == 0 || pp.nreal == 0) return;
  if (pp.nreal != nb) hipLaunchKernelGGL((k_halo_exchange<true>), dim3(nb), dim3(256), 0, st, *L, a, hx, pp);
  else hipLaunchKernelGGL((k_halo_exchange<false>), dim3(nb), dim3(256), 0, st, *L, a, hx, pp);
}
int mgxk_set_p2p_timeout(double ms) {
  const long long ticks = (long long)(ms * 1e5);
  return hipMemcpyToSymbol(HIP_SYMBOL(g_p2p_timeout_ticks), &ticks, sizeof ticks) == hipSuccess ? 0 : 1;
}
__global__ void k_err_to_double(const int *err, int extra, double *out) { out[0] = (err && *err != 0) || extra ? 1.0 : 0.0; }
void mgxk_err_to_double(hipStream_t st, const int *err, int extra, double *out) { hipLaunchKernelGGL(k_err_to_double, dim3(1), dim3(1), 0, st, err, extra, out); }
void mgxk_convert(hipStream_t st, const LevView *L, double *js, double *ref, int nslot, int slot, int dir) {
  const long long n = (long long)L->nz * (L->ny + 2) * (L->nx + 2);
  hipLaunchKernelGGL(k_convert, dim3((unsigned)((n + 255) / 256)), dim3(256), 0, st, *L, js, ref, nslot, slot, dir);
}
static int convert_tile(const LevView *L) {
  int tj = 128;
  while (tj > 16 && (size_t)tj * (L->nz + 1) * sizeof(double) > 150 * 1024) tj -= 16;
  return tj;
}
static void convert_slots(hipStream_t st, const LevView *L, const Slots8 &o, int ns, const double *ref) {
  const int tj = convert_tile(L);
  const size_t lds = (size_t)tj * (L->nz + 1) * sizeof(double);
  static bool attr = false;
  if (!attr) { if (hipFuncSetAttribute((const void *)k_convert_slots, hipFuncAttributeMaxDynamicSharedMemorySize, 160 * 1024) != hipSuccess) (void)hipGetLastError(); attr = true; }
  hipLaunchKernelGGL(k_convert_slots, dim3((L->ny + 2 + tj - 1) / tj, L->nx + 2, ns), dim3(256), lds, st, *L, o, ref, tj);
}
void mgxk_convert8(hipStream_t st, const LevView *L, const double *ref) {
  Slots8 o;
  for (int q = 0; q < 8; q++) o.s[q] = L->cA[q];
  convert_slots(st, L, o, 8, ref);
}
void mgxk_convert2(hipStream_t st, const LevView *L, double *out0, double *out1, const double *ref) {
  Slots8 o;
  for (int q = 0; q < 8; q++) o.s[q] = nullptr;
  o.s[0] = out0; o.s[1] = out1;
  convert_slots(st, L, o, 2, ref);
}
void mgxk_gather_place(hipStream_t st, const LevView *C, double *dstjs, const double *blk, int nxc, int nyc, int l, int m) {
  const long long n = (long long)C->nz * nyc * nxc;
  hipLaunchKernelGGL(k_gather_place, dim3((unsigned)((n + 255) / 256)), dim3(256), 0, st, *C, dstjs, blk, nxc, nyc, l, m);
}
void mgxk_block_to_ref(hipStream_t st, const LevView *Cs, const double *js, double *blk) {
  const long long n = (long long)Cs->nz * (Cs->ny + 2) * (Cs->nx + 2);
  hipLaunchKernelGGL(k_block_to_ref, dim3((unsigned)((n + 255) / 256)), dim3(256), 0, st, *Cs, js, blk);
}
void mgxk_gather_push(hipStream_t st, const LevView *Cs, const double *js, double *const *dst, unsigned long long *const *flags, int ng, int me,
                      unsigned long long seq, unsigned int *counter, int *err) {
  GatherP2P gp;
  for (int q = 0; q < 4; q++) { gp.dst[q] = q < ng ? dst[q] : nullptr; gp.flag[q] = q < ng ? flags[q] : nullptr; }
  gp.ng = ng; gp.me = me; gp.seq = seq; gp.counter = counter; gp.err = err;
  const long long n = (long long)Cs->nz * (Cs->ny + 2) * (Cs->nx + 2);
  long long nb = (n + 255) / 256;
  if (nb > 256) nb = 256;
  hipLaunchKernelGGL(k_gather_push, dim3((unsigned)nb), dim3(256), 0, st, *Cs, js, gp);
}
void mgxk_gather_place_wait(hipStream_t st, const LevView *C, double *dstjs, const double *blk, int nxc, int nyc, int l, int m,
                            unsigned long long *flag, unsigned long long seq, int *err) {
  const long long n = (long long)C->nz * nyc * nxc;
  long long nb = (n + 255) / 256;
  if (flag && nb > 128) nb = 128;
  hipLaunchKernelGGL(k_gather_place_wait, dim3((unsigned)nb), dim3(256), 0, st, *C, dstjs, blk, nxc, nyc, l, m, flag, seq, err);
}
void mgxk_split(hipStream_t st, const LevView *C, const LevView *Cs, const double *pc, double *dst, int l, int m) {
  const long long n = (long long)Cs->nz * (Cs->ny + 2) * (Cs->nx + 2);
  hipLaunchKernelGGL(k_split, dim3((unsigned)((n + 255) / 256)), dim3(256), 0, st, *C, *Cs, pc, dst, l, m);
}

}
```

### mgroms_amd/csrc/mgx_operator.h

```cpp
#pragma once
#include "mgx_device.h"

__device__ __forceinline__ void op_block_map(int gx, int gy, int &bx, int &by, int &bz) {
  const int per = gx * 2;
  int grp, local;
  if ((gy & 7) == 0) { const int xcd = blockIdx.x & 7; local = blockIdx.x >> 3; grp = xcd * (gy >> 3) + local / per; local -= (local / per) * per; }
  else { grp = blockIdx.x / per; local = blockIdx.x - grp * per; }
  by = grp; bz = local / gx; bx = local - bz * gx;
}

#define OP_BLOCK_SUM(acc, partial, idx)                                                                                                      \
  {                                                                                                                                          \
    for (int off = 32; off > 0; off >>= 1) acc += __shfl_down(acc, off, 64);                                                                 \
    __shared__ double red[16];                                                                                                               \
    const int tid = threadIdx.y * blockDim.x + threadIdx.x, w = tid >> 6;                                                                    \
    if ((tid & 63) == 0) red[w] = acc;                                                                                                       \
    __syncthreads();                                                                                                                         \
    if (tid == 0) {                                                                                                                          \
      double s = 0.0;                                                                                                                        \
      const int nw = (blockDim.x * blockDim.y + 63) >> 6;                                                                                    \
      for (int q = 0; q < nw; q++) s += red[q];                                                                                              \
      partial[idx] = s;                                                                                                                      \
    }                                                                                                                                        \
  }

#define OP_P(pl, ro, kr, pos) p[pl + ro + pos]
#define OP_P2(pl, ro, kr, pos, A, B) LD_PAIR(p + pl + ro + pos, A, B)
#define LOAD_ROW(PV, q, PJM, PIM, PC, A2, M3, M4, M5, N6, N7, N8)                                                                            \
  {                                                                                                                                          \
    const long long ro = (long long)((q)-1) * RS;                                                                                            \
    PJM = PV(o, ro, (q)-1, jm); PIM = PV(om, ro, (q)-1, c); PC = PV(o, ro, (q)-1, c); A2 = a2[o + ro + c];                                   \
    const double pj_ = PV(o, ro, (q)-1, jp), pi_ = PV(op, ro, (q)-1, c);                                                                     \
    M3 = a3[o + ro + jp] * pj_; M4 = a4[o + ro + jp] * pj_; M5 = a5[o + ro + jp] * pj_;                                                      \
    N6 = a6[op + ro + c] * pi_; N7 = a7[op + ro + c] * pi_; N8 = a8[op + ro + c] * pi_;                                                      \
  }
#define OP_COLUMN(PV, RHS, SINK)                                                                                                             \
  {                                                                                                                                          \
    const long long RS = L.RS;                                                                                                               \
    const int nz = L.nz;                                                                                                                     \
    const double *__restrict__ p = L.p;                                                                                                      \
    const double *__restrict__ a1 = L.cA[0], *__restrict__ a2 = L.cA[1], *__restrict__ a3 = L.cA[2],                                         \
                 *__restrict__ a4 = L.cA[3], *__restrict__ a5 = L.cA[4], *__restrict__ a6 = L.cA[5],                                         \
                 *__restrict__ a7 = L.cA[6], *__restrict__ a8 = L.cA[7];                                                                     \
    const long long o = (long long)i * L.plane, om = o - L.plane, op = o + L.plane;                                                          \
    double pjm_m, pjm_0, pjm_p, pim_m, pim_0, pim_p, pc_m, pc_0, pc_p, a2_0, a2_p;                                                           \
    double m3_m, m3_0, m4_0, m5_p, n6_m, n6_0, n7_0, n8_p, m3_p, m4_p, n6_p, n7_p;                                                           \
    double dum5, dum8;                                                                                                                       \
    LOAD_ROW(PV, 1, pjm_0, pim_0, pc_0, a2_0, m3_0, m4_0, dum5, n6_0, n7_0, dum8);                                                           \
    LOAD_ROW(PV, 2, pjm_p, pim_p, pc_p, a2_p, m3_p, m4_p, m5_p, n6_p, n7_p, n8_p);                                                           \
    (void)dum5; (void)dum8;                                                                                                                  \
                                                                                                                       \
    double rr = RHS(o + c) - a1[o + c] * pc_0 - a2_p * pc_p - a3[o + c] * pjm_p - a4[o + c] * pjm_0 - m4_0 - m5_p                            \
                - a6[o + c] * pim_p - a7[o + c] * pim_0 - n7_0 - n8_p;                                                                       \
    if (REAL)                                                                                                                                \
      rr = rr - a5[o + c] * PV(om, 0, 0, jp) - a5[op + jm] * PV(op, 0, 0, jm) - a8[o + c] * PV(om, 0, 0, jm) - a8[op + jp] * PV(op, 0, 0, jp); \
    const int jcol = jodd ? 2 * jh + 1 : 2 * jh + 2;                         \
    SINK(0, o + c, rr)                                                                                                                       \
    for (int k = 2; k <= nz - 1; k++) {                                                                                      \
      pjm_m = pjm_0; pjm_0 = pjm_p; pim_m = pim_0; pim_0 = pim_p; pc_m = pc_0; pc_0 = pc_p; a2_0 = a2_p;                                     \
      m3_m = m3_0; m3_0 = m3_p; m4_0 = m4_p; n6_m = n6_0; n6_0 = n6_p; n7_0 = n7_p;                                                          \
      LOAD_ROW(PV, k + 1, pjm_p, pim_p, pc_p, a2_p, m3_p, m4_p, m5_p, n6_p, n7_p, n8_p);                                                     \
      const long long ko = o + (long long)(k - 1) * RS + c;                                                                                  \
      rr = RHS(ko) - a1[ko] * pc_0 - a2_0 * pc_m - a2_p * pc_p - a3[ko] * pjm_p - m3_m - a4[ko] * pjm_0 - m4_0                               \
                   - a5[ko] * pjm_m - m5_p - a6[ko] * pim_p - n6_m - a7[ko] * pim_0 - n7_0 - a8[ko] * pim_m - n8_p;                          \
      SINK((long long)(k - 1) * RS, ko, rr)                                                                                                  \
    }                                                                                                                                        \
    {                                                                                                                 \
      pjm_m = pjm_0; pjm_0 = pjm_p; pim_m = pim_0; pim_0 = pim_p; pc_m = pc_0; pc_0 = pc_p; a2_0 = a2_p;                                     \
      m3_m = m3_0; m4_0 = m4_p; n6_m = n6_0; n7_0 = n7_p;                                                                                    \
      const long long ko = o + (long long)(nz - 1) * RS + c;                                                                                 \
      rr = RHS(ko) - a1[ko] * pc_0 - a2_0 * pc_m - m3_m - a4[ko] * pjm_0 - m4_0 - a5[ko] * pjm_m - n6_m                                      \
                   - a7[ko] * pim_0 - n7_0 - a8[ko] * pim_m;                                                                                 \
      SINK((long long)(nz - 1) * RS, ko, rr)                                                                                                 \
    }                                                                                                                                        \
  }

#define LOAD_WIN(PV, PV2, q, PC, PJM, PIM, PJP, PIP, ZY, ZX, A2)                                                                                      \
  { const long long ro = (long long)(((q) <= nz ? (q) : nz) - 1) * RS;                                                                       \
    const int kr = ((q) <= nz ? (q) : nz) - 1;                                                                                               \
    PC = PV(o, ro, kr, c); PV2(o, ro, kr, jm, PJM, PJP) PIM = PV(om, ro, kr, c); PIP = PV(op, ro, kr, c);                                    \
    ZY = *(zy + o + ro + c); ZX = *(zx + o + ro + c); A2 = ld_rt(a2 + o + ro + c, stream); }
#define LOAD_ROWV(RHS_LOAD, q, ZYJM, ZYJP, ZXIM, ZXIP, A4O, A4JP, A7O, A7IP, BK)                                                             \
  { const long long ro = (long long)(((q) <= nz ? (q) : nz) - 1) * RS, ko = o + ro + c;                                                      \
    LD_PAIR(zy + o + ro + jm, ZYJM, ZYJP) ZXIM = zx[om + ro + c]; ZXIP = zx[op + ro + c];                                                    \
    A4O = *(a4 + ko); A4JP = a4[o + ro + jp]; A7O = *(a7 + ko); A7IP = a7[op + ro + c]; BK = RHS_LOAD(ko); }
#define OP_COLUMN_MF(PV, PV2, RHS_LOAD, SINK)                                                                                                 \
  {                                                                                                                                          \
    const long long RS = L.RS;                                                                                                               \
    const int nz = L.nz;                                                                                                                     \
    const double *__restrict__ p = L.p;                                                                                                      \
    const double *__restrict__ a1 = L.cA[0], *__restrict__ a2 = L.cA[1], *__restrict__ a4 = L.cA[3], *__restrict__ a5 = L.cA[4],             \
                 *__restrict__ a7 = L.cA[6], *__restrict__ a8 = L.cA[7], *__restrict__ zy = L.zy, *__restrict__ zx = L.zx;                   \
    const long long o = (long long)i * L.plane, om = o - L.plane, op = o + L.plane;                                                          \
    const double qrt = 0.25;                                                                                                                 \
     \
      \
                      \
    double pc_m = 0, pc_0, pc_p, pc_n, pjm_m = 0, pjm_0, pjm_p, pjm_n, pim_m = 0, pim_0, pim_p, pim_n, pjp_m = 0, pjp_0, pjp_p, pjp_n, pip_m = 0, pip_0, pip_p, pip_n; \
    double zy_m = 0, zy_0, zy_p, zy_n, zx_m = 0, zx_0, zx_p, zx_n, a2_0, a2_p, a2_n;                                                         \
    double zyjm, zyjp, zxim, zxip, a4o, a4jp, a7o, a7ip, bk, zyjm_n, zyjp_n, zxim_n, zxip_n, a4o_n, a4jp_n, a7o_n, a7ip_n, bk_n;             \
     \
    const double d_first = a1[o + c], d_last = a1[o + (long long)(nz - 1) * RS + c];                                                         \
    double e0 = 0, e1 = 0, e2 = 0, e3 = 0, e4 = 0, e5 = 0, e6 = 0, e7 = 0;                                                                   \
    if (REAL) { e0 = a5[o + c]; e1 = PV(om, 0, 0, jp); e2 = a5[op + jm]; e3 = PV(op, 0, 0, jm); e4 = a8[o + c]; e5 = PV(om, 0, 0, jm); e6 = a8[op + jp]; e7 = PV(op, 0, 0, jp); } \
    LOAD_WIN(PV, PV2, 1, pc_0, pjm_0, pim_0, pjp_0, pip_0, zy_0, zx_0, a2_0)                                                                          \
    LOAD_ROWV(RHS_LOAD, 1, zyjm, zyjp, zxim, zxip, a4o, a4jp, a7o, a7ip, bk)                                                                 \
    LOAD_WIN(PV, PV2, 2, pc_p, pjm_p, pim_p, pjp_p, pip_p, zy_p, zx_p, a2_p)                                                                 \
    for (int k = 1; k <= nz; k++) {                                                                                                          \
      const long long ro = (long long)(k - 1) * RS, ko = o + ro + c;                                                                         \
      LOAD_WIN(PV, PV2, k + 2, pc_n, pjm_n, pim_n, pjp_n, pip_n, zy_n, zx_n, a2_n)                                                           \
      LOAD_ROWV(RHS_LOAD, k + 1, zyjm_n, zyjp_n, zxim_n, zxip_n, a4o_n, a4jp_n, a7o_n, a7ip_n, bk_n)                                         \
      double rr;                                                                                                                             \
      if (k == 1) {                                                                                                                          \
        rr = bk - d_first * pc_0 - a2_p * pc_p - (qrt * (zy_p + zyjm)) * pjm_p - a4o * pjm_0 - a4jp * pjp_0                                  \
                   - (-qrt * (zyjp + zy_p)) * pjp_p - (qrt * (zx_p + zxim)) * pim_p - a7o * pim_0 - a7ip * pip_0                             \
                   - (-qrt * (zxip + zx_p)) * pip_p;                                                                                         \
        if (REAL) rr = rr - e0 * e1 - e2 * e3 - e4 * e5 - e6 * e7;                                                                           \
      } else if (k < nz) {                                                                                                                   \
        const double c3 = qrt * (zy_p + zyjm), c3m = qrt * (zyjp + zy_m), c5 = -qrt * (zy_m + zyjm), c5m = -qrt * (zyjp + zy_p);             \
        const double c6 = qrt * (zx_p + zxim), c6m = qrt * (zxip + zx_m), c8 = -qrt * (zx_m + zxim), c8m = -qrt * (zxip + zx_p);             \
        const double dk = -a2_0 - a2_p - a4o - a4jp - a7o - a7ip - c6 - c6m - c8 - c8m - c3 - c3m - c5 - c5m;   \
        rr = bk - dk * pc_0 - a2_0 * pc_m - a2_p * pc_p - c3 * pjm_p - c3m * pjp_m                                                           \
                   - a4o * pjm_0 - a4jp * pjp_0 - c5 * pjm_m - c5m * pjp_p                                                                   \
                   - c6 * pim_p - c6m * pip_m - a7o * pim_0 - a7ip * pip_0                                                                   \
                   - c8 * pim_m - c8m * pip_p;                                                                                               \
      } else {                                                                                                                               \
        rr = bk - d_last * pc_0 - a2_0 * pc_m - (qrt * (zyjp + zy_m)) * pjp_m - a4o * pjm_0 - a4jp * pjp_0                                   \
                   - (-qrt * (zy_m + zyjm)) * pjm_m - (qrt * (zxip + zx_m)) * pip_m - a7o * pim_0 - a7ip * pip_0                             \
                   - (-qrt * (zx_m + zxim)) * pim_m;                                                                                         \
      }                                                                                                                                      \
      SINK(ro, ko, rr)                                                                                                                       \
      pc_m = pc_0; pc_0 = pc_p; pc_p = pc_n; pjm_m = pjm_0; pjm_0 = pjm_p; pjm_p = pjm_n; pim_m = pim_0; pim_0 = pim_p; pim_p = pim_n;       \
      pjp_m = pjp_0; pjp_0 = pjp_p; pjp_p = pjp_n; pip_m = pip_0; pip_0 = pip_p; pip_p = pip_n;                                              \
      zy_m = zy_0; zy_0 = zy_p; zy_p = zy_n; zx_m = zx_0; zx_0 = zx_p; zx_p = zx_n; a2_0 = a2_p; a2_p = a2_n;                                \
      zyjm = zyjm_n; zyjp = zyjp_n; zxim = zxim_n; zxip = zxip_n; a4o = a4o_n; a4jp = a4jp_n; a7o = a7o_n; a7ip = a7ip_n; bk = bk_n;         \
    }                                                                                                                                        \
  }
```

### mgroms_amd/csrc/mgx_relax_common.h

```cpp
#pragma once
#include "mgx_device.h"

#define XCD_BLOCK_MAP(nunit, gx, bx, ig)                                             \
  {                                                                                  \
    if (gx < 0) { gx = -gx; ig = blockIdx.x / gx; bx = blockIdx.x - ig * gx; }       \
    else if ((nunit & 7) == 0) {                                                     \
      const int xcd = blockIdx.x & 7, local = blockIdx.x >> 3;                       \
      ig = xcd * (nunit >> 3) + local / gx;                                          \
      bx = local - (local / gx) * gx;                                                \
    } else { ig = blockIdx.x / gx; bx = blockIdx.x - ig * gx; }                      \
  }

#define MF_NB_LOAD(q)                                                                                     \
  if ((q) <= NZ) {                                                                                        \
    const long long ro_ = (long long)((q)-1) * RS; const int s_ = (q) % RN;                               \
    if (PAIR) LD_PAIR(p + o + ro_ + jm, r_pjm[s_], r_pjp[s_]) else r_pjm[s_] = p[o + ro_ + jm];           \
    r_pim[s_] = p[om + ro_ + c];                                                                          \
    if (!PAIR) r_pjp[s_] = p[o + ro_ + jp];                                                               \
    r_pip[s_] = p[op + ro_ + c];                                                                          \
    if (PAIR) LD_PAIR(zy + o + ro_ + jm, r_zyjm[s_], r_zyjp[s_])                                          \
    else { r_zyjm[s_] = *(zy + o + ro_ + jm); r_zyjp[s_] = *(zy + o + ro_ + jp); }                        \
    r_zxim[s_] = *(zx + om + ro_ + c); r_zxip[s_] = *(zx + op + ro_ + c);                                 \
    if (!ZW) { r_a4[s_] = *(a4 + o + ro_ + jp); r_a7[s_] = *(a7 + op + ro_ + c); }                        \
  }
#define MF_OW_LOAD(q)                                                                                     \
  if ((q) <= NZ) {                                                                                        \
    const long long ko_ = o + (long long)((q)-1) * RS + c; const int s_ = (q) % RO;                       \
    o_b[s_] = ld_stream<ST>(b + ko_); o_a2[s_] = ld_stream<ST>(a2 + ko_);                                 \
    if (!ZW) { o_a4[s_] = ld_stream<ST>(a4 + ko_); o_a7[s_] = ld_stream<ST>(a7 + ko_); }                  \
    if (!ZG) { o_zy[ZG ? 0 : s_] = ld_stream<ST>(zy + ko_); o_zx[ZG ? 0 : s_] = ld_stream<ST>(zx + ko_); } \
  }
#define ZR_GEN(kk, q) ({ const double z0_ = cffr[(kk)-1] + csr[(kk)-1] * hh[q]; z0_ * hh[q] * hv[q] + hz[q] * (1. + z0_ * hv[q]); })
#define OWN_SLOPES(kk, ZY, ZX) { const double zn1_ = ZR_GEN(kk, 1), zn2_ = ZR_GEN(kk, 2), zn3_ = ZR_GEN(kk, 3), zn4_ = ZR_GEN(kk, 4); \
    ZY = DIVC(hlf * (zn2_ - zn1_), gdy, rdy) * gdx; ZX = DIVC(hlf * (zn4_ - zn3_), gdx, rdx) * gdy; }
#define ZW_GEN(kk, q) ({ const double z0_ = cffw[(kk)-1] + csw[(kk)-1] * hh[q]; z0_ * hh[q] * hv[q] + hz[q] * (1. + z0_ * hv[q]); })

#define MF_PROLOGUE(XN, GN)                                                                                     \
  const long long RS = L.RS;                                                                              \
  double *__restrict__ p = L.p;                                                                           \
  const double *__restrict__ b = L.b;                                                                     \
  const double *__restrict__ a1 = L.cA[0], *__restrict__ a2 = L.cA[1], *__restrict__ a4 = L.cA[3], *__restrict__ a5 = L.cA[4], \
               *__restrict__ a7 = L.cA[6], *__restrict__ a8 = L.cA[7], *__restrict__ bet = L.bet,                    \
               *__restrict__ zy = L.zy, *__restrict__ zx = L.zx;                                          \
  const long long o = (long long)i * L.plane, om = o - L.plane, op = o + L.plane;                         \
  const double qrt = 0.25, hlf = 0.5;                                                                     \
  constexpr int RN = D + 2;   \
  constexpr int RO = D + 2;                     \
  double r_pjm[RN], r_pim[RN], r_pjp[RN], r_pip[RN], r_zyjm[RN], r_zyjp[RN], r_zxim[RN], r_zxip[RN], r_a4[RN], r_a7[RN]; \
  double o_b[RO], o_a2[RO], o_a4[RO], o_a7[RO], o_zy[ZG ? 1 : RO], o_zx[ZG ? 1 : RO];                     \
  double x[XN], g[GN];       \
  const int lane = threadIdx.x;                                                                           \
                                                          \
  const double dg1 = a1[o + c], dgn = a1[o + (long long)(NZ - 1) * RS + c];                               \
   \
   \
   \
  double zw0[5], zw1[5], hh[5], hv[5], hz[5];                                                             \
  const double *__restrict__ cffw = L.cffw, *__restrict__ csw = L.csw, *__restrict__ cffr = L.cffr, *__restrict__ csr = L.csr; \
  double r4c = 0, r4p = 0, r7c = 0, r7p = 0, gdx = 1, gdy = 1, rdx = 0, rdy = 0;                          \
  double a4_1 = 0, a4j_1 = 0, a7_1 = 0, a7i_1 = 0, a4_n = 0, a4j_n = 0, a7_n = 0, a7i_n = 0;              \
  double m4c = 0, m4p = 0, d4c = 1, d4p = 1, m7c = 0, m7p = 0, d7c = 1, d7p = 1;                          \
  if (ZW) {                                                                                               \
    const long long rn = (long long)(NZ - 1) * RS;                                                        \
    a4_1 = a4[o + c]; a4j_1 = a4[o + jp]; a7_1 = a7[o + c]; a7i_1 = a7[op + c];                           \
    a4_n = a4[o + rn + c]; a4j_n = a4[o + rn + jp]; a7_n = a7[o + rn + c]; a7i_n = a7[op + rn + c];       \
    const long long q2 = (long long)i * RS;                                                               \
    m4c = L.m4[q2 + c]; m4p = L.m4[q2 + jp]; d4c = L.d4[q2 + c]; d4p = L.d4[q2 + jp];                     \
    m7c = L.m7[q2 + c]; m7p = L.m7[q2 + RS + c]; d7c = L.d7[q2 + c]; d7p = L.d7[q2 + RS + c];             \
    const long long cq[5] = {q2 + c, q2 + jm, q2 + jp, q2 - RS + c, q2 + RS + c};   \
    _Pragma("unroll") for (int q = 0; q < 5; q++) { hh[q] = L.h2[cq[q]]; hv[q] = L.hi2[cq[q]]; hz[q] = L.ze2[cq[q]]; } \
    r4c = RCP_REF(d4c); r4p = RCP_REF(d4p); r7c = RCP_REF(d7c); r7p = RCP_REF(d7p);                       \
    if (ZG) { gdx = L.dx2[q2 + c]; gdy = L.dy2[q2 + c]; rdx = RCP_REF(gdx); rdy = RCP_REF(gdy); }         \
  }                                                                                                       \
   \
  double d1 = 0, d2 = 0, d3 = 0, d4 = 0, e1 = 0, e2 = 0, e3 = 0, e4 = 0;                                  \
  if (REAL) {                                                                                             \
    const double *__restrict__ q1 = SNAP ? L.p1 : p;                                                      \
    const long long s = SNAP ? (long long)i * RS : o, sm = SNAP ? s - RS : om, sp = SNAP ? s + RS : op;   \
    d1 = q1[sm + jp]; d2 = q1[sp + jm]; d3 = q1[sm + jm]; d4 = q1[sp + jp];                               \
    e1 = a5[o + c]; e2 = a5[op + jm]; e3 = a8[o + c]; e4 = a8[op + jp];                                   \
  }                                                                                                       \
  _Pragma("unroll") for (int q = 1; q <= 1 + D; q++) { MF_NB_LOAD(q) }                                    \
  _Pragma("unroll") for (int q = 1; q <= 1 + D; q++) { MF_OW_LOAD(q) }                                    \
                   \
  double pjm_m = 0, pjm_0 = r_pjm[1 % RN], pjm_p = 0, pim_m = 0, pim_0 = r_pim[1 % RN], pim_p = 0;        \
  double pjp_m = 0, pjp_0 = r_pjp[1 % RN], pjp_p = 0, pip_m = 0, pip_0 = r_pip[1 % RN], pip_p = 0;        \
  double zy_m = 0, zy_0 = 0, zy_p = 0, zx_m = 0, zx_0 = 0, zx_p = 0;                                      \
  if (ZG) OWN_SLOPES(1, zy_0, zx_0)                                                                       \
  else { zy_0 = o_zy[ZG ? 0 : 1 % RO]; zx_0 = o_zx[ZG ? 0 : 1 % RO]; }                                    \
  double xv = 0.0, betp = 0.0;

#define MF_ROW(k)                                                                                         \
  {                                                                                                       \
    MF_NB_LOAD(k + 1 + D)                                                                                 \
    MF_OW_LOAD(k + 1 + D)                                                                                 \
    if (k < NZ) {                                                                                         \
      const int s1 = (k + 1) % RN, t1 = (k + 1) % RO;                                                     \
      pjm_p = r_pjm[s1]; pim_p = r_pim[s1]; pjp_p = r_pjp[s1]; pip_p = r_pip[s1];                         \
      if (ZG) OWN_SLOPES(k + 1, zy_p, zx_p)                                                               \
      else { zy_p = o_zy[ZG ? 0 : t1]; zx_p = o_zx[ZG ? 0 : t1]; }                                        \
    }                                                                                                     \
    const int s = k % RO, n = k % RN;                                                                     \
    const double zyjm = r_zyjm[n], zyjp = r_zyjp[n], zxim = r_zxim[n], zxip = r_zxip[n];                  \
     \
                                                                            \
    const double c3 = qrt * (zy_p + zyjm), c3m = qrt * (zyjp + zy_m), c5 = -qrt * (zy_m + zyjm), c5m = -qrt * (zyjp + zy_p); \
    const double c6 = qrt * (zx_p + zxim), c6m = qrt * (zxip + zx_m), c8 = -qrt * (zx_m + zxim), c8m = -qrt * (zxip + zx_p); \
    double a4o, a4jp, a7o, a7ip;            \
    if (!ZW) { a4o = o_a4[s]; a4jp = r_a4[n]; a7o = o_a7[s]; a7ip = r_a7[n]; }                            \
    else if (k == 1) { a4o = a4_1; a4jp = a4j_1; a7o = a7_1; a7ip = a7i_1; }                              \
    else if (k == NZ) { a4o = a4_n; a4jp = a4j_n; a7o = a7_n; a7ip = a7i_n; }                             \
    else {                                                                                                \
      if (k == 2) { _Pragma("unroll") for (int q = 0; q < 5; q++) zw0[q] = ZW_GEN(2, q); }                \
      _Pragma("unroll") for (int q = 0; q < 5; q++) zw1[q] = ZW_GEN(k + 1, q);                            \
      const double wo0 = zw0[0], wop1 = zw1[0];                                                           \
      a4o = DIVC(qrt * (wop1 - wo0 + zw1[1] - zw0[1]) * m4c, d4c, r4c);                                   \
      a4jp = DIVC(qrt * (zw1[2] - zw0[2] + wop1 - wo0) * m4p, d4p, r4p);                                  \
      a7o = DIVC(qrt * (wop1 - wo0 + zw1[3] - zw0[3]) * m7c, d7c, r7c);                                   \
      a7ip = DIVC(qrt * (zw1[4] - zw0[4] + wop1 - wo0) * m7p, d7p, r7p);                                  \
      _Pragma("unroll") for (int q = 0; q < 5; q++) zw0[q] = zw1[q];                                      \
    }                                                                                                     \
    double dk, betk;                                                     \
    if (k == 1) dk = dg1;                                                                                 \
    else if (k == NZ) dk = dgn;                                                                           \
    else dk = -o_a2[s] - o_a2[(k + 1) % RO] - a4o - a4jp - a7o - a7ip - c6 - c6m - c8 - c8m - c3 - c3m - c5 - c5m; \
    if (k == 1) betk = 1.0 / dk;                                                                          \
    else { const double gk = o_a2[s] * betp; MF_G_PUT(k, gk) betk = 1.0 / (dk - o_a2[s] * gk); }          \
    betp = betk;                                                                                          \
    double rhs;                                                                                           \
    if (k == 1) {                                                                                         \
      rhs = o_b[s] - c3 * pjm_p - a4o * pjm_0 - a4jp * pjp_0 - c5m * pjp_p                                \
                   - c6 * pim_p - a7o * pim_0 - a7ip * pip_0 - c8m * pip_p;                               \
      if (REAL) rhs = rhs - e1 * d1 - e2 * d2 - e3 * d3 - e4 * d4;                                        \
      xv = rhs * betk;                                                                                    \
    } else if (k < NZ) {                                                                                  \
      rhs = o_b[s] - c3 * pjm_p - c3m * pjp_m - a4o * pjm_0 - a4jp * pjp_0                                \
                   - c5 * pjm_m - c5m * pjp_p                                                             \
                   - c6 * pim_p - c6m * pip_m - a7o * pim_0 - a7ip * pip_0                                \
                   - c8 * pim_m - c8m * pip_p;                                                            \
      xv = (rhs - o_a2[s] * xv) * betk;                                                                   \
    } else {                                                                                              \
      rhs = o_b[s] - c3m * pjp_m - a4o * pjm_0 - a4jp * pjp_0 - c5 * pjm_m                                \
                   - c6m * pip_m - a7o * pim_0 - a7ip * pip_0 - c8 * pim_m;                               \
      xv = (rhs - o_a2[s] * xv) * betk;                                                                   \
    }                                                                                                     \
    MF_X_PUT(k, xv, o_a2[s], betk)                                                                        \
    pjm_m = pjm_0; pjm_0 = pjm_p; pim_m = pim_0; pim_0 = pim_p;                                           \
    pjp_m = pjp_0; pjp_0 = pjp_p; pip_m = pip_0; pip_0 = pip_p;                                           \
    zy_m = zy_0; zy_0 = zy_p; zx_m = zx_0; zx_0 = zx_p;                                                   \
  }

#define SC_NB_LOAD(q)                                                            \
  if ((q) <= NZ) {                                                               \
    const long long ro_ = (long long)((q)-1) * RS; const int s_ = (q) % RN;      \
    r_pjm[s_] = p[o + ro_ + jm]; r_pim[s_] = p[om + ro_ + c];                    \
    r_pjp[s_] = p[o + ro_ + jp]; r_pip[s_] = p[op + ro_ + c];                    \
    r_a3[s_] = a3[o + ro_ + jp]; r_a4[s_] = a4[o + ro_ + jp]; r_a5[s_] = a5[o + ro_ + jp]; \
    r_a6[s_] = a6[op + ro_ + c]; r_a7[s_] = a7[op + ro_ + c]; r_a8[s_] = a8[op + ro_ + c]; \
  }
#define SC_OW_LOAD(q)                                                            \
  if ((q) <= NZ) {                                                               \
    const long long ko_ = o + (long long)((q)-1) * RS + c; const int s_ = (q) % RO; \
    o_b[s_] = ld_stream<ST>(b + ko_); o_a2[s_] = ld_stream<ST>(a2 + ko_); o_a3[s_] = ld_stream<ST>(a3 + ko_); o_a4[s_] = ld_stream<ST>(a4 + ko_); o_a5[s_] = ld_stream<ST>(a5 + ko_); \
    o_a6[s_] = ld_stream<ST>(a6 + ko_); o_a7[s_] = ld_stream<ST>(a7 + ko_); o_a8[s_] = ld_stream<ST>(a8 + ko_); o_bet[s_] = ld_stream<ST>(bet + ko_); \
  }
#define SC_NB_USE(q, PJM, PIM, M3, M4, M5, N6, N7, N8)                           \
  { const int s_ = (q) % RN; PJM = r_pjm[s_]; PIM = r_pim[s_];                   \
    M3 = r_a3[s_] * r_pjp[s_]; M4 = r_a4[s_] * r_pjp[s_]; M5 = r_a5[s_] * r_pjp[s_]; \
    N6 = r_a6[s_] * r_pip[s_]; N7 = r_a7[s_] * r_pip[s_]; N8 = r_a8[s_] * r_pip[s_]; }

#define SC_PROLOGUE(XN, GN)                                                                               \
  const long long RS = L.RS;                                                                              \
  double *__restrict__ p = L.p;                                                                           \
  const double *__restrict__ b = L.b;                                                                     \
  const double *__restrict__ a2 = L.cA[1], *__restrict__ a3 = L.cA[2], *__restrict__ a4 = L.cA[3],        \
               *__restrict__ a5 = L.cA[4], *__restrict__ a6 = L.cA[5], *__restrict__ a7 = L.cA[6],        \
               *__restrict__ a8 = L.cA[7], *__restrict__ bet = L.bet;                                     \
  const long long o = (long long)i * L.plane, om = o - L.plane, op = o + L.plane;                         \
  constexpr int RN = D + 1;                                             \
  constexpr int RO = D + 1;                                                   \
  double r_pjm[RN], r_pim[RN], r_pjp[RN], r_pip[RN], r_a3[RN], r_a4[RN], r_a5[RN], r_a6[RN], r_a7[RN], r_a8[RN]; \
  double o_b[RO], o_a2[RO], o_a3[RO], o_a4[RO], o_a5[RO], o_a6[RO], o_a7[RO], o_a8[RO], o_bet[RO];        \
  double x[XN], g[GN];       \
   \
  double d1 = 0, d2 = 0, d3 = 0, d4 = 0, e1 = 0, e2 = 0, e3 = 0, e4 = 0;                                  \
  if (REAL) {                                                                                             \
    const double *__restrict__ q1 = SNAP ? L.p1 : p;                                                      \
    const long long s = SNAP ? (long long)i * RS : o, sm = SNAP ? s - RS : om, sp = SNAP ? s + RS : op;   \
    d1 = q1[sm + jp]; d2 = q1[sp + jm]; d3 = q1[sm + jm]; d4 = q1[sp + jp];                               \
    e1 = a5[o + c]; e2 = a5[op + jm]; e3 = a8[o + c]; e4 = a8[op + jp];                                   \
  }                                                                                                       \
                                                             \
  _Pragma("unroll") for (int q = 1; q <= 1 + D; q++) { SC_NB_LOAD(q) }                                    \
  _Pragma("unroll") for (int q = 1; q <= D; q++) { SC_OW_LOAD(q) }                                        \
  double pjm_m = 0, pjm_0, pjm_p, pim_m = 0, pim_0, pim_p;                                                \
  double m3_m = 0, m3_0, m4_0, m5_p, n6_m = 0, n6_0, n7_0, n8_p, m3_p, m4_p, n6_p, n7_p, dum5, dum8;      \
  SC_NB_USE(1, pjm_0, pim_0, m3_0, m4_0, dum5, n6_0, n7_0, dum8)                                          \
  (void)dum5; (void)dum8;                                                                                 \
  double xv = 0.0, betp = 0.0;

#define SC_ROW(k)                                                                                         \
  {                                                                                                       \
                                                                              \
    SC_NB_LOAD(k + 1 + D)                                                                                 \
    SC_OW_LOAD(k + D)                                                                                     \
    if (k < NZ) { SC_NB_USE(k + 1, pjm_p, pim_p, m3_p, m4_p, m5_p, n6_p, n7_p, n8_p) }                    \
    const int s = k % RO;                                                                                 \
    double rhs;                                                                                           \
     \
    if (k > 1) SC_G_PUT(k, o_a2[s] * betp)                                                                \
    betp = o_bet[s];                                                                                      \
    if (k == 1) {                                                                                         \
      rhs = o_b[s] - o_a3[s] * pjm_p - o_a4[s] * pjm_0 - m4_0 - m5_p - o_a6[s] * pim_p - o_a7[s] * pim_0 - n7_0 - n8_p; \
      if (REAL) rhs = rhs - e1 * d1 - e2 * d2 - e3 * d3 - e4 * d4;                                        \
      xv = rhs * o_bet[s];                                                                                \
    } else if (k < NZ) {                                                                                  \
      rhs = o_b[s] - o_a3[s] * pjm_p - m3_m - o_a4[s] * pjm_0 - m4_0 - o_a5[s] * pjm_m - m5_p             \
                   - o_a6[s] * pim_p - n6_m - o_a7[s] * pim_0 - n7_0 - o_a8[s] * pim_m - n8_p;            \
      xv = (rhs - o_a2[s] * xv) * o_bet[s];                                                               \
    } else {                                                                                              \
      rhs = o_b[s] - m3_m - o_a4[s] * pjm_0 - m4_0 - o_a5[s] * pjm_m - n6_m - o_a7[s] * pim_0 - n7_0 - o_a8[s] * pim_m; \
      xv = (rhs - o_a2[s] * xv) * o_bet[s];                                                               \
    }                                                                                                     \
    SC_X_PUT(k, xv)                                                                                       \
                                                                         \
    pjm_m = pjm_0; pjm_0 = pjm_p; pim_m = pim_0; pim_0 = pim_p;                                           \
    m3_m = m3_0; m3_0 = m3_p; m4_0 = m4_p; n6_m = n6_0; n6_0 = n6_p; n7_0 = n7_p;                         \
  }
```

### mgroms_amd/csrc/mgx_resrest.hip

```cpp
#include "mgx_switches.h"
#include "mgx_device.h"

namespace {

struct RowW {
  double P[4];
  double Pm[2];
  double Pp[2];
  double ZY4[4];
  double ZX[2];
  double A2[2];
};
struct RowR {
  double ZXm[2];
  double ZXp[2];
  double A4[3];
  double A7[2];
  double A7p[2];
  double B[2];
};

struct Geo {
  long long o, om, op;
  int c[4];
};

#define LD_PAIR(ptr, A, B) { double2 t2_; __builtin_memcpy(&t2_, (ptr), 16); A = t2_.x; B = t2_.y; }
__device__ __forceinline__ void load_w(RowW &w, const LevView &F, const Geo &g, const long long ro) {
  const double *__restrict__ p = F.p, *__restrict__ zy = F.zy, *__restrict__ zx = F.zx, *__restrict__ a2 = F.cA[1];
  LD_PAIR(p + g.o + ro + g.c[0], w.P[0], w.P[2])
  LD_PAIR(p + g.o + ro + g.c[1], w.P[1], w.P[3])
  LD_PAIR(zy + g.o + ro + g.c[0], w.ZY4[0], w.ZY4[2])
  LD_PAIR(zy + g.o + ro + g.c[1], w.ZY4[1], w.ZY4[3])
#pragma unroll
  for (int jj = 0; jj < 2; jj++) {
    const long long e = g.o + ro + g.c[jj + 1];
    w.Pm[jj] = p[g.om + ro + g.c[jj + 1]]; w.Pp[jj] = p[g.op + ro + g.c[jj + 1]];
    w.ZX[jj] = zx[e]; w.A2[jj] = a2[e];
  }
}

__device__ __forceinline__ void load_r(RowR &r, const LevView &F, const Geo &g, const long long ro) {
  const double *__restrict__ b = F.b, *__restrict__ zx = F.zx, *__restrict__ a4 = F.cA[3], *__restrict__ a7 = F.cA[6];
  LD_PAIR(a4 + g.o + ro + g.c[1], r.A4[0], r.A4[2])
  r.A4[1] = a4[g.o + ro + g.c[2]];
#pragma unroll
  for (int jj = 0; jj < 2; jj++) {
    const int c = g.c[jj + 1];
    r.ZXm[jj] = zx[g.om + ro + c]; r.ZXp[jj] = zx[g.op + ro + c];
    r.A7[jj] = a7[g.o + ro + c]; r.A7p[jj] = a7[g.op + ro + c];
    r.B[jj] = b[g.o + ro + c];
  }
}

}

template <bool REAL, int AW, int AR, bool NORM = false>
__global__ __launch_bounds__(256, 1) void k_residual_restrict(LevView F, LevView C, double *__restrict__ dst, Sides ph, double *__restrict__ zero, int gx, int gy,
                                                             double *__restrict__ partial = nullptr, double *__restrict__ dup = nullptr) {
  __shared__ double red_ss[4];
  double ss = 0.0;
  int bx, by;
  if ((gy & 7) == 0) { const int xcd = blockIdx.x & 7, local = blockIdx.x >> 3; by = xcd * (gy >> 3) + local / gx; bx = local - (local / gx) * gx; }
  else { by = blockIdx.x / gx; bx = blockIdx.x - by * gx; }
  const int half = threadIdx.x >> 5;
  int j2 = 1 + bx * 32 + (threadIdx.x & 31);
  const int i2 = 1 + by * blockDim.y + threadIdx.y;
  if (i2 > C.nx) {
    if (NORM) { if ((threadIdx.x & 63) == 0) red_ss[threadIdx.y] = 0.0; __syncthreads(); if (threadIdx.x == 0 && threadIdx.y == 0) partial[blockIdx.x] = red_ss[0] + red_ss[1] + red_ss[2] + red_ss[3]; }
    return;
  }
  const bool live = j2 <= C.ny;
  if (!live) j2 = C.ny;
  const int nz = F.nz;
  const long long RS = F.RS;
  Geo g;
  g.o = (long long)(2 * i2 - 1 + half) * F.plane; g.om = g.o - F.plane; g.op = g.o + F.plane;
  g.c[1] = F.HO + (j2 - 1); g.c[2] = F.EO + j2; g.c[0] = F.EO + (j2 - 1); g.c[3] = F.HO + j2;
  const double qrt = 0.25;
  const double *__restrict__ a1 = F.cA[0], *__restrict__ a5 = F.cA[4], *__restrict__ a8 = F.cA[7];

  double dlast[2];
#pragma unroll
  for (int jj = 0; jj < 2; jj++) dlast[jj] = a1[g.o + (long long)(nz - 1) * RS + g.c[jj + 1]];
  double dedge[2], e[2][8];
#pragma unroll
  for (int jj = 0; jj < 2; jj++) {
    const int c = g.c[jj + 1], jm = g.c[jj], jp = g.c[jj + 2];
    dedge[jj] = a1[g.o + c];
    if (REAL) {
      e[jj][0] = a5[g.o + c]; e[jj][1] = F.p[g.om + jp]; e[jj][2] = a5[g.op + jm]; e[jj][3] = F.p[g.op + jm];
      e[jj][4] = a8[g.o + c]; e[jj][5] = F.p[g.om + jm]; e[jj][6] = a8[g.op + jp]; e[jj][7] = F.p[g.op + jp];
    }
  }
  constexpr int NWB = 3 + AW, NRB = 1 + AR;
  constexpr int U = (NWB % NRB == 0) ? NWB : NWB * NRB;
  static_assert(U <= 12, "unroll");
  RowW W[NWB];
  RowR R[NRB];
#pragma unroll
  for (int q = 0; q < AW + 2; q++) load_w(W[q], F, g, (long long)(q + 1 <= nz ? q : nz - 1) * RS);
  load_r(R[NRB - 1], F, g, 0);
#pragma unroll
  for (int q = 0; q < AR - 1; q++) load_r(R[q], F, g, (long long)(q + 2 <= nz ? q + 1 : nz - 1) * RS);
  double z = 0.0;
  const long long oc = (long long)i2 * C.plane + jpos(C, j2);

#define RR_LOADS(k, Wn, Rn)                                                                                                 \
    load_w(Wn, F, g, (long long)((k) + 1 + AW <= nz ? (k) + AW : nz - 1) * RS);                                              \
    load_r(Rn, F, g, (long long)((k) + AR <= nz ? (k) + AR - 1 : nz - 1) * RS);
#define RR_CELL_IN(Wm, W0, Wp, R0)                                                                                          \
      const double pc_m = Wm.P[jj + 1], pc_0 = W0.P[jj + 1], pc_p = Wp.P[jj + 1];                                            \
      const double pjm_m = Wm.P[jj], pjm_0 = W0.P[jj], pjm_p = Wp.P[jj];                                                     \
      const double pjp_m = Wm.P[jj + 2], pjp_0 = W0.P[jj + 2], pjp_p = Wp.P[jj + 2];                                         \
      const double pim_m = Wm.Pm[jj], pim_0 = W0.Pm[jj], pim_p = Wp.Pm[jj];                                                  \
      const double pip_m = Wm.Pp[jj], pip_0 = W0.Pp[jj], pip_p = Wp.Pp[jj];                                                  \
      const double zy_m = Wm.ZY4[jj + 1], zy_p = Wp.ZY4[jj + 1], zx_m = Wm.ZX[jj], zx_p = Wp.ZX[jj];                         \
      const double zyjm = W0.ZY4[jj], zyjp = W0.ZY4[jj + 2];                                                                \
      const double zxim = R0.ZXm[jj], zxip = R0.ZXp[jj];                                                                    \
      const double a4o = R0.A4[jj], a4jp = R0.A4[jj + 1], a7o = R0.A7[jj], a7ip = R0.A7p[jj];                                \
      const double a2_0 = W0.A2[jj], a2_p = Wp.A2[jj];                                                                      \
      const double c3 = qrt * (zy_p + zyjm), c3m = qrt * (zyjp + zy_m), c5 = -qrt * (zy_m + zyjm), c5m = -qrt * (zyjp + zy_p); \
      const double c6 = qrt * (zx_p + zxim), c6m = qrt * (zxip + zx_m), c8 = -qrt * (zx_m + zxim), c8m = -qrt * (zxip + zx_p); \
      (void)pc_m; (void)pjm_m; (void)pjp_m; (void)pim_m; (void)pip_m; (void)c3m; (void)c5; (void)c6m; (void)c8; (void)a2_0;
#define RR_SUM(k, r)                                                                                                        \
    if (NORM && live) ss = ss + (r[0] * r[0] + r[1] * r[1]);                                                                \
    const double rA_B = __shfl_xor(r[0], 32, 64), rB_B = __shfl_xor(r[1], 32, 64);                                          \
    if ((k) & 1) z = r[0] + rA_B + r[1] + rB_B;                                                                             \
    else {                                                                                                                  \
      z = z + r[0] + rA_B + r[1] + rB_B;                                                                                    \
      if (half == 0 && live) {                                                                                              \
        const long long rc = (long long)(((k) >> 1) - 1) * C.RS;                                                            \
        dst[oc + rc] = z;                                                                                                   \
        mirror_store(C, dst, rc, j2, i2, jpos(C, j2), z, ph);                                                               \
        if (dup) { dup[oc + rc] = z; mirror_store(C, dup, rc, j2, i2, jpos(C, j2), z, ph); }                                 \
        if (zero) { zero[oc + rc] = 0.0; mirror_store(C, zero, rc, j2, i2, jpos(C, j2), 0.0, ph); }                          \
      }                                                                                                                     \
    }
#define RR_GENERAL(rr, R0)                                                                                                  \
      {                                                                                                                     \
        const double dk = -a2_0 - a2_p - a4o - a4jp - a7o - a7ip - c6 - c6m - c8 - c8m - c3 - c3m - c5 - c5m;               \
        rr = R0.B[jj] - dk * pc_0 - a2_0 * pc_m - a2_p * pc_p - c3 * pjm_p - c3m * pjp_m                                    \
                      - a4o * pjm_0 - a4jp * pjp_0 - c5 * pjm_m - c5m * pjp_p                                                \
                      - c6 * pim_p - c6m * pip_m - a7o * pim_0 - a7ip * pip_0                                                \
                      - c8 * pim_m - c8m * pip_p;                                                                            \
      }
#define RR_LAST(rr, R0)                                                                                                     \
      {                                                                                                                     \
        rr = R0.B[jj] - dlast[jj] * pc_0 - a2_0 * pc_m - c3m * pjp_m - a4o * pjm_0 - a4jp * pjp_0                           \
                      - c5 * pjm_m - c6m * pip_m - a7o * pim_0 - a7ip * pip_0 - c8 * pim_m;                                  \
      }
#define RR_STEP(k, Wm, W0, Wp, Wn, R0, Rn)                                                                                  \
  {                                                                                                                         \
    RR_LOADS(k, Wn, Rn)                                                                                                     \
    double r[2];                                                                                                            \
    _Pragma("unroll") for (int jj = 0; jj < 2; jj++) {                                                                     \
      RR_CELL_IN(Wm, W0, Wp, R0)                                                                                            \
      double rr;                                                                                                            \
      if ((k) < nz) RR_GENERAL(rr, R0)                                                                                       \
      else RR_LAST(rr, R0)                                                                                                  \
      r[jj] = rr;                                                                                                           \
    }                                                                                                                       \
    RR_SUM(k, r)                                                                                                            \
  }
  {
    RR_LOADS(1, W[AW + 2], R[AR - 1])
    double r[2];
#pragma unroll
    for (int jj = 0; jj < 2; jj++) {
      RR_CELL_IN(W[0], W[0], W[1], R[NRB - 1])
      double rr = R[NRB - 1].B[jj] - dedge[jj] * pc_0 - a2_p * pc_p - c3 * pjm_p - a4o * pjm_0 - a4jp * pjp_0
                                   - c5m * pjp_p - c6 * pim_p - a7o * pim_0 - a7ip * pip_0 - c8m * pip_p;
      if (REAL) rr = rr - e[jj][0] * e[jj][1] - e[jj][2] * e[jj][3] - e[jj][4] * e[jj][5] - e[jj][6] * e[jj][7];
      r[jj] = rr;
    }
    RR_SUM(1, r)
  }
  int k = 2;
  for (; k + U - 1 <= nz; k += U) {
#pragma unroll
    for (int q = 0; q < U; q++) RR_STEP(k + q, W[q % NWB], W[(q + 1) % NWB], W[(q + 2) % NWB], W[(q + 2 + AW) % NWB], R[q % NRB], R[(q + AR) % NRB])
  }
#pragma unroll
  for (int q = 0; q < U - 1; q++) {
    if (k + q <= nz) RR_STEP(k + q, W[q % NWB], W[(q + 1) % NWB], W[(q + 2) % NWB], W[(q + 2 + AW) % NWB], R[q % NRB], R[(q + AR) % NRB])
  }
#undef RR_STEP
#undef RR_LOADS
  if (NORM) {
#pragma unroll
    for (int off = 32; off > 0; off >>= 1) ss += __shfl_xor(ss, off, 64);
    if ((threadIdx.x & 63) == 0) red_ss[threadIdx.y] = ss;
    __syncthreads();
    if (threadIdx.x == 0 && threadIdx.y == 0) partial[blockIdx.x] = red_ss[0] + red_ss[1] + red_ss[2] + red_ss[3];
  }
}

template <bool REAL, int S, bool NORM = false>
__global__ __launch_bounds__(64) void k_residual_restrict_flat(LevView F, LevView C, double *__restrict__ dst, Sides ph, double *__restrict__ zero, int gx,
                                                              double *__restrict__ partial = nullptr, double *__restrict__ dup = nullptr) {
  double ss = 0.0;
  const int nz = F.nz, nks = (nz + S - 1) / S, ng = gx * C.nx;
  int grp, ks;
  if ((ng & 7) == 0) { const int xcd = blockIdx.x & 7, local = blockIdx.x >> 3; ks = local % nks; grp = xcd * (ng >> 3) + local / nks; }
  else { ks = blockIdx.x % nks; grp = blockIdx.x / nks; }
  const int i2 = 1 + grp / gx, bx = grp - (grp / gx) * gx;
  const int half = threadIdx.x >> 5;
  int j2 = 1 + bx * 32 + (threadIdx.x & 31);
  const bool live = j2 <= C.ny;
  if (!live) j2 = C.ny;
  const int k = ks * S + 1;
  const long long RS = F.RS;
  Geo g;
  g.o = (long long)(2 * i2 - 1 + half) * F.plane; g.om = g.o - F.plane; g.op = g.o + F.plane;
  g.c[1] = F.HO + (j2 - 1); g.c[2] = F.EO + j2; g.c[0] = F.EO + (j2 - 1); g.c[3] = F.HO + j2;
  const double qrt = 0.25;
  const double *__restrict__ a1 = F.cA[0], *__restrict__ a5 = F.cA[4], *__restrict__ a8 = F.cA[7];
  RowW W[S + 2];
  RowR R[S];
#pragma unroll
  for (int r = 0; r < S + 2; r++) {
    const int kr = k - 1 + r < 1 ? 1 : (k - 1 + r > nz ? nz : k - 1 + r);
    load_w(W[r], F, g, (long long)(kr - 1) * RS);
  }
#pragma unroll
  for (int r = 0; r < S; r++) {
    const int kr = k + r > nz ? nz : k + r;
    load_r(R[r], F, g, (long long)(kr - 1) * RS);
  }
  double dedge[2] = {0.0, 0.0}, e[2][8];
  if (k == 1) {
#pragma unroll
    for (int jj = 0; jj < 2; jj++) {
      const int c = g.c[jj + 1], jm = g.c[jj], jp = g.c[jj + 2];
      dedge[jj] = a1[g.o + c];
      if (REAL) {
        e[jj][0] = a5[g.o + c]; e[jj][1] = F.p[g.om + jp]; e[jj][2] = a5[g.op + jm]; e[jj][3] = F.p[g.op + jm];
        e[jj][4] = a8[g.o + c]; e[jj][5] = F.p[g.om + jm]; e[jj][6] = a8[g.op + jp]; e[jj][7] = F.p[g.op + jp];
      }
    }
  }
  double dlast[2] = {0.0, 0.0};
  if (k + S > nz) {
#pragma unroll
    for (int jj = 0; jj < 2; jj++) dlast[jj] = a1[g.o + (long long)(nz - 1) * RS + g.c[jj + 1]];
  }
  double z = 0.0;
  const long long oc = (long long)i2 * C.plane + jpos(C, j2);
#pragma unroll
  for (int r = 0; r < S; r++) {
    const int kr = k + r;
    if (kr <= nz) {
      double rv[2];
#pragma unroll
      for (int jj = 0; jj < 2; jj++) {
        RR_CELL_IN(W[r], W[r + 1], W[r + 2], R[r])
        double rr;
        if (r == 0 && kr == 1) {
          rr = R[r].B[jj] - dedge[jj] * pc_0 - a2_p * pc_p - c3 * pjm_p - a4o * pjm_0 - a4jp * pjp_0
                          - c5m * pjp_p - c6 * pim_p - a7o * pim_0 - a7ip * pip_0 - c8m * pip_p;
          if (REAL) rr = rr - e[jj][0] * e[jj][1] - e[jj][2] * e[jj][3] - e[jj][4] * e[jj][5] - e[jj][6] * e[jj][7];
        } else if (kr < nz) RR_GENERAL(rr, R[r])
        else RR_LAST(rr, R[r])
        rv[jj] = rr;
      }
      RR_SUM(kr, rv)
    }
  }
  if (NORM) {
#pragma unroll
    for (int off = 32; off > 0; off >>= 1) ss += __shfl_xor(ss, off, 64);
    if (threadIdx.x == 0) partial[blockIdx.x] = ss;
  }
}
#undef RR_SUM
#undef RR_CELL_IN
#undef RR_GENERAL
#undef RR_LAST

extern "C" {

int mgxk_residual_restrict_grid(const LevView *F, const LevView *C) {
  const int gx = (C->ny + 31) / 32;
  if ((long long)F->nx * F->ny * F->nz <= mgx_switches().resrest_flat_max) {
    const int Sv = (mgx_switches().resrest_flat_s >= 4 && F->nz >= 4) ? 4 : 2;
    return gx * C->nx * ((F->nz + Sv - 1) / Sv);
  }
  return gx * ((C->nx + 3) / 4);
}
int mgxk_residual_restrict_ex(hipStream_t st, const LevView *F, const LevView *C, double *dst, int real, Sides ph, double *zero, double *partial, double *dup) {
  mgx_before_launch();
  const Switches &sw = mgx_switches();
  if (sw.no_resrest || F->zy == nullptr || F->nz < 2 || (F->nz & 1)) return 0;
  if (C->nx * 2 != F->nx || C->ny * 2 != F->ny) return 0;
  if ((long long)F->nx * F->ny * F->nz < sw.resrest_min) return 0;
  if ((long long)F->nx * F->ny * F->nz <= sw.resrest_flat_max) {
    const int gx = (C->ny + 31) / 32, Sr = sw.resrest_flat_s ? sw.resrest_flat_s : 2;
    dim3 blk(WAVE);
#define RRF(REALV, SV, NV) hipLaunchKernelGGL((k_residual_restrict_flat<REALV, SV, NV>), dim3((unsigned)gx * C->nx * ((F->nz + SV - 1) / SV)), blk, 0, st, *F, *C, dst, ph, zero, gx, partial, dup)
#define RRF2(SV) { if (partial) { if (real) RRF(true, SV, true); else RRF(false, SV, true); } else { if (real) RRF(true, SV, false); else RRF(false, SV, false); } }
    if (Sr >= 4 && F->nz >= 4) RRF2(4) else RRF2(2)
#undef RRF2
#undef RRF
    return mgx_launched();
  }
  const int by = 4, gx = (C->ny + 31) / 32, gy = (C->nx + by - 1) / by;
  dim3 blk(WAVE, by), grd(gx * gy);
  const int deep = sw.resrest_ahead;
#define RRW(REALV, AWV, ARV, NV) hipLaunchKernelGGL((k_residual_restrict<REALV, AWV, ARV, NV>), grd, blk, 0, st, *F, *C, dst, ph, zero, gx, gy, partial, dup)
#define RRW2(AWV, ARV) { if (partial) { if (real) RRW(true, AWV, ARV, true); else RRW(false, AWV, ARV, true); } else { if (real) RRW(true, AWV, ARV, false); else RRW(false, AWV, ARV, false); } }
  switch (deep) {
    case 12: RRW2(1, 2) break;
    case 21: RRW2(2, 1) break;
    default: RRW2(1, 1) break;
  }
#undef RRW2
#undef RRW
  return mgx_launched();
}
int mgxk_residual_restrict(hipStream_t st, const LevView *F, const LevView *C, double *dst, int real, Sides ph, double *zero) {
  return mgxk_residual_restrict_ex(st, F, C, dst, real, ph, zero, nullptr, nullptr);
}

}
```

### mgroms_amd/csrc/mgx_switches.cpp

```cpp
#include "mgx_switches.h"
#include <cstdlib>

namespace {

enum Rule { SET_TRUE, SET_FALSE, ATOI, ATOLL };
struct Row {
  const char *env; bool Switches::*flag; int Switches::*num; long long Switches::*wide; Rule rule; long long dflt; const char *what;
  Row(const char *e, bool Switches::*m, Rule r, long long d, const char *w) : env(e), flag(m), num(nullptr), wide(nullptr), rule(r), dflt(d), what(w) {}
  Row(const char *e, int Switches::*m, Rule r, long long d, const char *w) : env(e), flag(nullptr), num(m), wide(nullptr), rule(r), dflt(d), what(w) {}
  Row(const char *e, long long Switches::*m, Rule r, long long d, const char *w) : env(e), flag(nullptr), num(nullptr), wide(m), rule(r), dflt(d), what(w) {}
};
const Row TABLE[] = {
  {"MGX_NO_XCD",                 &Switches::no_xcd,                SET_TRUE,  0,                "plain block order instead of the per-XCD block map of the colour passes (relax, tall, k-split); same bits"},
  {"MGX_NO_REG",                 &Switches::no_reg,                SET_TRUE,  0,                "small closed levels without the one-thread-per-column kernel (k_relax_reg): the LDS-resident or the generic one; same bits"},
  {"MGX_NO_TINY",                &Switches::no_tiny,               SET_TRUE,  0,                "small closed levels without the all-in-LDS kernel (k_relax_tiny); same bits"},
  {"MGX_NO_WAVE",                &Switches::no_wave,               SET_TRUE,  0,                "the two coarsest levels without the wave kernels (k_relax_wave, four and eight waves included): the older one-workgroup kernels; same bits"},
  {"MGX_NO_WAVE_FUSE",           &Switches::no_wave_fuse,          SET_TRUE,  0,                "coarse2fine / residual + fine2coarse as launches of their own around the coarse relax instead of folded into it; same bits"},
  {"MGX_NO_TALL",                &Switches::no_tall,               SET_TRUE,  0,                "generic colour pass at nz = 80, 96, 128 instead of the tall-column pass (and no chained snapshots there); same bits"},
  {"MGX_NO_KS",                  &Switches::no_ks,                 SET_TRUE,  0,                "row-by-row colour passes on the mid levels instead of every k-split kernel (pass, colour pair, persistent relax); same bits"},
  {"MGX_NO_KS8",                 &Switches::ks8,                   SET_FALSE, 1,                "nz = 8 levels: row-by-row instead of the k-split colour pass; same bits"},
  {"MGX_NO_KS64",                &Switches::ks64,                  SET_FALSE, 1,                "nz = 64 levels that fit the caches: row-by-row instead of the k-split colour pass; same bits"},
  {"MGX_NO_KS2",                 &Switches::no_ks2,                SET_TRUE,  0,                "four colours on the closed mid levels: one launch per colour instead of per colour pair (and no persistent relax); same bits"},
  {"MGX_NO_KSP",                 &Switches::no_ksp,                SET_TRUE,  0,                "one launch per colour pair instead of the persistent relax; also presets option \"ksp\", which cannot turn it back on; same bits"},
  {"MGX_KSP_SC1",                &Switches::ksp_fence,             SET_FALSE, 1,                "the persistent relax hands planes over with sc1 accesses instead of release / acquire fences (measured on gfx950 only); same bits"},
  {"MGX_KS_NW",                  &Switches::ks_nw,                 ATOI,      0,                "= 4: four waves per workgroup instead of eight in the k-split colour pass; same bits"},
  {"MGX_RBSEQ_D0_KERNEL",        &Switches::rbseq_d0_kernel,       SET_TRUE,  0,                "sequential-order red-black: the walk reads d0 on every level, written by the colour pass or by k_rbseq_d0, instead of forming it on narrow half-rows; same bits"},
  {"MGX_RBSEQ_NO_D0_MID",        &Switches::rbseq_d0_mid,          SET_FALSE, 1,                "half-rows of 65..128 columns: the walk forms d0 itself instead of reading what the colour pass left (same expression; no test pins the bits)"},
  {"MGX_NO_RBSEQ_WALK_APPLY",    &Switches::no_rbseq_walk_apply,   SET_TRUE,  0,                "small levels: walk and correction by the scan kernels instead of k_rbseq_walk_apply; same bits"},
  {"MGX_RBSEQ_WINDOW_NO_XMAP",   &Switches::rbseq_window_no_xmap,  SET_TRUE,  0,                "plain block order instead of the per-XCD block map of the windowed walk; same bits"},
  {"MGX_RBW_PRIO",               &Switches::rbw_prio,              ATOI,      1,                "= 0: the walking wave of the windowed walk at normal priority instead of s_setprio 3; same bits"},
  {"MGX_C2F_KC",                 &Switches::c2f_kc,                ATOI,      0,                "> 0: that many coarse levels per lane in the prolongation instead of 16 (before the cut for small levels); same bits"},
  {"MGX_C2F_NT",                 &Switches::c2f_nt,                ATOI,      -1,               ">= 0: the prolongation's streaming hints forced on (1) or off (0) instead of chosen by the level's size; same bits"},
  {"MGX_NO_RESREST",             &Switches::no_resrest,            SET_TRUE,  0,                "residual and restriction as two kernels instead of the fused one; same bits"},
  {"MGX_RESREST_MIN",            &Switches::resrest_min,           ATOLL,     0,                "the fused residual + restriction only from that many fine cells on, two kernels below; same bits"},
  {"MGX_RESREST_FLAT_MAX",       &Switches::resrest_flat_max,      ATOLL,     256LL * 256 * 64, "fine cells up to which the fused residual + restriction takes its flat form (no walk up the column); same bits"},
  {"MGX_RESREST_FLAT_S",         &Switches::resrest_flat_s,        ATOI,      0,                ">= 4: four fine rows per wave in the flat form instead of two; same bits"},
  {"MGX_RESREST_AHEAD",          &Switches::resrest_ahead,         ATOI,      11,               "10 * AW + AR, the look-ahead of the walking form: 12 and 21 are instantiated beside 11; same bits"},
  {"MGX_P2P_MAXBLK",             &Switches::p2p_maxblk,            ATOI,      128,              "block cap of the halo push kernel (its grid must stay resident beside a neighbour's smoother); same bits"},
  {"MGX_P2P_IPT",                &Switches::p2p_ipt,               ATOI,      1,                "test hook: at least that many items per thread in the halo push kernel; same bits"},
  {"MGX_MODEL_KR",               &Switches::model_kr,              ATOI,      0,                "> 0 (A/B and test hook): runs of exactly that many rows in the flux kernels and correct_uvw; same bits"},
};

}

const Switches &mgx_switches() {
  static const Switches sw = [] {
    Switches s = {};
    for (const Row &r : TABLE) {
      const char *e = getenv(r.env);
      if (r.flag) s.*r.flag = e ? r.rule == SET_TRUE : r.dflt != 0;
      else if (r.num) s.*r.num = e ? atoi(e) : (int)r.dflt;
      else s.*r.wide = e ? atoll(e) : r.dflt;
    }
    return s;
  }();
  return sw;
}
```

### mgroms_amd/csrc/mgx_switches.h

```cpp
#pragma once

struct Switches {
  bool no_xcd;
  bool no_reg, no_tiny, no_wave, no_wave_fuse;
  bool no_tall;
  bool no_ks, ks8, ks64, no_ks2, no_ksp, ksp_fence;
  int ks_nw;
  bool rbseq_d0_kernel, rbseq_d0_mid, no_rbseq_walk_apply, rbseq_window_no_xmap;
  int rbw_prio;
  int c2f_kc, c2f_nt;
  bool no_resrest;
  long long resrest_min, resrest_flat_max;
  int resrest_flat_s, resrest_ahead;
  int p2p_maxblk, p2p_ipt, model_kr;
};

const Switches &mgx_switches();
```

Before: 523.9 V-cycles/s (x number of 512x512x64 blocks when N>1: weak scaling).

## Generate matrix slots 4 and 7 from depth formula in fused residual-restrict; double-double norms

In the walking fused residual+restriction kernel (down leg, no norm), the interior rows of coefficient slots 4 and 7 are recomputed from per-column depth data (h, hi, ze, cffw/csw, m/d factors) instead of being streamed from HBM. The last row's values are parked in LDS and exchanged across lanes with bpermute. Separately, residual norm reductions switch to compensated double-double accumulation, which doubles the partial buffer and adds some reduction work. The recomputation trades HBM traffic for extra FLOPs, register pressure and LDS use.

```diff
diff --git a/mgroms_amd/csrc/mgx_define.cpp b/mgroms_amd/csrc/mgx_define.cpp
--- a/mgroms_amd/csrc/mgx_define.cpp
+++ b/mgroms_amd/csrc/mgx_define.cpp
@@ -416,7 +416,7 @@
     if (np > max_part) max_part = np;
   }
   S.npartial = (int)max_part;
-  CHK(dmalloc(&S.d_partial, max_part));
+  CHK(dmalloc(&S.d_partial, 2 * max_part));
   CHK(dmalloc(&S.d_scalar, 8));
   if (S.method == M_RB && S.real) CHK(dmalloc(&S.rho_dev, 32));
   HIPCHK(hipHostMalloc((void **)&S.h_scalar, 8 * sizeof(double)));
diff --git a/mgroms_amd/csrc/mgx_device.h b/mgroms_amd/csrc/mgx_device.h
--- a/mgroms_amd/csrc/mgx_device.h
+++ b/mgroms_amd/csrc/mgx_device.h
@@ -56,11 +56,23 @@
 static inline void mgx_before_launch() { const hipError_t e = hipGetLastError(); if (e != hipSuccess && mgx_pending_error == hipSuccess) mgx_pending_error = e; }
 static inline int mgx_launched() { return hipGetLastError() == hipSuccess ? 1 : 0; }
 
+__device__ __forceinline__ void dd_add(double &hi, double &lo, const double t) {
+  const double s = hi + t, bb = s - hi;
+  lo = lo + ((hi - (s - bb)) + (t - bb));
+  hi = s;
+}
+__device__ __forceinline__ void dd_merge(double &hi, double &lo, const double ohi, const double olo) {
+  const double s = hi + ohi, bb = s - hi;
+  lo = (lo + olo) + ((hi - (s - bb)) + (ohi - bb));
+  hi = s;
+}
+
 static inline dim3 col_grid(int ncol_half, int nplanes, int z = 1) { return dim3((ncol_half + WAVE - 1) / WAVE, (nplanes + 3) / 4, z); }
 
 #define RCP_REF(b) ({ const double b_ = (b); double r_ = __builtin_amdgcn_rcp(b_); double e_ = __builtin_fma(-b_, r_, 1.0); r_ = __builtin_fma(r_, e_, r_); \
                       e_ = __builtin_fma(-b_, r_, 1.0); __builtin_fma(r_, e_, r_); })
 #define DIVC(a, b, rb) ({ const double a_ = (a); const double q_ = a_ * (rb); const double e_ = __builtin_fma(-(b), q_, a_); __builtin_fma(e_, (rb), q_); })
+#define ZW_GEN(kk, q) ({ const double z0_ = cffw[(kk)-1] + csw[(kk)-1] * hh[q]; z0_ * hh[q] * hv[q] + hz[q] * (1. + z0_ * hv[q]); })
 #define LD_PAIR(ptr, A, B) { double2 t2_; __builtin_memcpy(&t2_, (ptr), 16); A = t2_.x; B = t2_.y; }
 
 __device__ __forceinline__ double wave_shr1(double x) {
diff --git a/mgroms_amd/csrc/mgx_kernels.hip b/mgroms_amd/csrc/mgx_kernels.hip
--- a/mgroms_amd/csrc/mgx_kernels.hip
+++ b/mgroms_amd/csrc/mgx_kernels.hip
@@ -2,7 +2,7 @@
 #include "mgx_operator.h"
 
 #define RES_RHS(ko) b[ko]
-#define RES_SINK(ro, ko, rr) { r[ko] = rr; mirror_store(L, r, ro, jcol, i, c, rr, ph); acc = acc + rr * rr; }
+#define RES_SINK(ro, ko, rr) { r[ko] = rr; mirror_store(L, r, ro, jcol, i, c, rr, ph); dd_add(acc, acl, rr * rr); }
 template <bool REAL>
 __global__ __launch_bounds__(256) void k_residual(LevView L, double *__restrict__ partial, int want_norm, int gx, int gy, Sides ph, int stream) {
   int bx, by, bz;
@@ -10,7 +10,7 @@
   const int jh = bx * WAVE + threadIdx.x;
   const int i = 1 + by * blockDim.y + threadIdx.y;
   const int jodd = bz == 0;
-  double acc = 0.0;
+  double acc = 0.0, acl = 0.0;
   if (jh < (L.ny >> 1) && i <= L.nx) {
     int c, jm, jp;
     COL_POS(L, jh, jodd, c, jm, jp)
@@ -19,11 +19,11 @@
     OP_COLUMN(OP_P, RES_RHS, RES_SINK)
   }
   if (!want_norm) return;
-  OP_BLOCK_SUM(acc, partial, blockIdx.x)
+  OP_BLOCK_SUM_DD(acc, acl, partial, blockIdx.x, gridDim.x)
 }
 
 #define RES_RHS_MF(ko) ld_rt(b + ko, stream)
-#define RES_SINK_MF(ro, ko, rr) { st_rt(r + ko, rr, stream); mirror_store(L, r, ro, jodd ? 2 * jh + 1 : 2 * jh + 2, i, c, rr, ph); acc = acc + rr * rr; }
+#define RES_SINK_MF(ro, ko, rr) { st_rt(r + ko, rr, stream); mirror_store(L, r, ro, jodd ? 2 * jh + 1 : 2 * jh + 2, i, c, rr, ph); dd_add(acc, acl, rr * rr); }
 template <bool REAL>
 __global__ __launch_bounds__(256) void k_residual_mf(LevView L, double *__restrict__ partial, int want_norm, int gx, int gy, Sides ph, int stream) {
   int bx, by, bz;
@@ -31,7 +31,7 @@
   const int jh = bx * WAVE + threadIdx.x;
   const int i = 1 + by * blockDim.y + threadIdx.y;
   const int jodd = bz == 0;
-  double acc = 0.0;
+  double acc = 0.0, acl = 0.0;
   if (jh < (L.ny >> 1) && i <= L.nx) {
     int c, jm, jp;
     COL_POS(L, jh, jodd, c, jm, jp)
@@ -40,7 +40,7 @@
     OP_COLUMN_MF(OP_P, OP_P2, RES_RHS_MF, RES_SINK_MF)
   }
   if (!want_norm) return;
-  OP_BLOCK_SUM(acc, partial, blockIdx.x)
+  OP_BLOCK_SUM_DD(acc, acl, partial, blockIdx.x, gridDim.x)
 }
 
 __global__ __launch_bounds__(256) void k_sumsq(LevView L, const double *__restrict__ a, double *__restrict__ partial) {
@@ -78,6 +78,22 @@
     __syncthreads();
   }
   if (threadIdx.x == 0) out[0] = red[0];
+}
+
+__global__ __launch_bounds__(256) void k_reduce_partials_dd(const double *__restrict__ partial, int n, double *__restrict__ out) {
+  __shared__ double red[512];
+  double s = 0.0, sl = 0.0;
+  for (int q = threadIdx.x; q < n; q += 256) dd_merge(s, sl, partial[q], partial[n + q]);
+  red[threadIdx.x] = s; red[256 + threadIdx.x] = sl;
+  __syncthreads();
+  for (int off = 128; off > 0; off >>= 1) {
+    if ((int)threadIdx.x < off) {
+      dd_merge(s, sl, red[threadIdx.x + off], red[256 + threadIdx.x + off]);
+      red[threadIdx.x] = s; red[256 + threadIdx.x] = sl;
+    }
+    __syncthreads();
+  }
+  if (threadIdx.x == 0) out[0] = s + sl;
 }
 
 struct LevChain { LevView v[5]; };
@@ -597,9 +613,9 @@
     else hipLaunchKernelGGL((k_residual_mf<false>), grd, blk, 0, st, *L, partial, want_norm, gx, gy, ph, level_streams(L));
   } else if (real) hipLaunchKernelGGL((k_residual<true>), grd, blk, 0, st, *L, partial, want_norm, gx, gy, ph, level_streams(L));
   else hipLaunchKernelGGL((k_residual<false>), grd, blk, 0, st, *L, partial, want_norm, gx, gy, ph, level_streams(L));
-  if (want_norm) hipLaunchKernelGGL(k_reduce_partials, dim3(1), dim3(256), 0, st, partial, (int)grd.x, out);
-}
-void mgxk_reduce(hipStream_t st, const double *partial, int n, double *out) { hipLaunchKernelGGL(k_reduce_partials, dim3(1), dim3(256), 0, st, partial, n, out); }
+  if (want_norm) hipLaunchKernelGGL(k_reduce_partials_dd, dim3(1), dim3(256), 0, st, partial, (int)grd.x, out);
+}
+void mgxk_reduce(hipStream_t st, const double *partial, int n, double *out) { hipLaunchKernelGGL(k_reduce_partials_dd, dim3(1), dim3(256), 0, st, partial, n, out); }
 void mgxk_sumsq(hipStream_t st, const LevView *L, const double *a, double *partial, double *out) {
   dim3 blk(WAVE, 4), grd = col_grid(L->ny / 2, L->nx, 2);
   hipLaunchKernelGGL(k_sumsq, grd, blk, 0, st, *L, a, partial);
diff --git a/mgroms_amd/csrc/mgx_operator.h b/mgroms_amd/csrc/mgx_operator.h
--- a/mgroms_amd/csrc/mgx_operator.h
+++ b/mgroms_amd/csrc/mgx_operator.h
@@ -21,6 +21,21 @@
       const int nw = (blockDim.x * blockDim.y + 63) >> 6;                                                                                    \
       for (int q = 0; q < nw; q++) s += red[q];                                                                                              \
       partial[idx] = s;                                                                                                                      \
+    }                                                                                                                                        \
+  }
+
+#define OP_BLOCK_SUM_DD(acc, acl, partial, idx, n)                                                                                           \
+  {                                                                                                                                          \
+    for (int off = 32; off > 0; off >>= 1) { const double oh_ = __shfl_down(acc, off, 64), ol_ = __shfl_down(acl, off, 64); dd_merge(acc, acl, oh_, ol_); } \
+    __shared__ double red[32];                                                                                                               \
+    const int tid = threadIdx.y * blockDim.x + threadIdx.x, w = tid >> 6;                                                                    \
+    if ((tid & 63) == 0) { red[w] = acc; red[16 + w] = acl; }                                                                                \
+    __syncthreads();                                                                                                                         \
+    if (tid == 0) {                                                                                                                          \
+      double s = 0.0, sl = 0.0;                                                                                                              \
+      const int nw = (blockDim.x * blockDim.y + 63) >> 6;                                                                                    \
+      for (int q = 0; q < nw; q++) dd_merge(s, sl, red[q], red[16 + q]);                                                                     \
+      partial[idx] = s; partial[(n) + (idx)] = sl;                                                                                           \
     }                                                                                                                                        \
   }
 
diff --git a/mgroms_amd/csrc/mgx_relax_common.h b/mgroms_amd/csrc/mgx_relax_common.h
--- a/mgroms_amd/csrc/mgx_relax_common.h
+++ b/mgroms_amd/csrc/mgx_relax_common.h
@@ -33,7 +33,6 @@
 #define ZR_GEN(kk, q) ({ const double z0_ = cffr[(kk)-1] + csr[(kk)-1] * hh[q]; z0_ * hh[q] * hv[q] + hz[q] * (1. + z0_ * hv[q]); })
 #define OWN_SLOPES(kk, ZY, ZX) { const double zn1_ = ZR_GEN(kk, 1), zn2_ = ZR_GEN(kk, 2), zn3_ = ZR_GEN(kk, 3), zn4_ = ZR_GEN(kk, 4); \
     ZY = DIVC(hlf * (zn2_ - zn1_), gdy, rdy) * gdx; ZX = DIVC(hlf * (zn4_ - zn3_), gdx, rdx) * gdy; }
-#define ZW_GEN(kk, q) ({ const double z0_ = cffw[(kk)-1] + csw[(kk)-1] * hh[q]; z0_ * hh[q] * hv[q] + hz[q] * (1. + z0_ * hv[q]); })
 
 #define MF_PROLOGUE(XN, GN)                                                                                     \
   const long long RS = L.RS;                                                                              \
diff --git a/mgroms_amd/csrc/mgx_resrest.hip b/mgroms_amd/csrc/mgx_resrest.hip
--- a/mgroms_amd/csrc/mgx_resrest.hip
+++ b/mgroms_amd/csrc/mgx_resrest.hip
@@ -25,7 +25,6 @@
   int c[4];
 };
 
-#define LD_PAIR(ptr, A, B) { double2 t2_; __builtin_memcpy(&t2_, (ptr), 16); A = t2_.x; B = t2_.y; }
 __device__ __forceinline__ void load_w(RowW &w, const LevView &F, const Geo &g, const long long ro) {
   const double *__restrict__ p = F.p, *__restrict__ zy = F.zy, *__restrict__ zx = F.zx, *__restrict__ a2 = F.cA[1];
   LD_PAIR(p + g.o + ro + g.c[0], w.P[0], w.P[2])
@@ -40,26 +39,46 @@
   }
 }
 
+template <bool ZW = false>
 __device__ __forceinline__ void load_r(RowR &r, const LevView &F, const Geo &g, const long long ro) {
   const double *__restrict__ b = F.b, *__restrict__ zx = F.zx, *__restrict__ a4 = F.cA[3], *__restrict__ a7 = F.cA[6];
-  LD_PAIR(a4 + g.o + ro + g.c[1], r.A4[0], r.A4[2])
-  r.A4[1] = a4[g.o + ro + g.c[2]];
+  if (!ZW) {
+    LD_PAIR(a4 + g.o + ro + g.c[1], r.A4[0], r.A4[2])
+    r.A4[1] = a4[g.o + ro + g.c[2]];
+  }
 #pragma unroll
   for (int jj = 0; jj < 2; jj++) {
     const int c = g.c[jj + 1];
     r.ZXm[jj] = zx[g.om + ro + c]; r.ZXp[jj] = zx[g.op + ro + c];
-    r.A7[jj] = a7[g.o + ro + c]; r.A7p[jj] = a7[g.op + ro + c];
+    if (!ZW) { r.A7[jj] = a7[g.o + ro + c]; r.A7p[jj] = a7[g.op + ro + c]; }
     r.B[jj] = b[g.o + ro + c];
   }
 }
-
-}
-
-template <bool REAL, int AW, int AR, bool NORM = false>
+__device__ __forceinline__ void load_s(RowR &r, const LevView &F, const Geo &g, const long long ro) {
+  const double *__restrict__ a4 = F.cA[3], *__restrict__ a7 = F.cA[6];
+  LD_PAIR(a4 + g.o + ro + g.c[1], r.A4[0], r.A4[2])
+  r.A4[1] = a4[g.o + ro + g.c[2]];
+#pragma unroll
+  for (int jj = 0; jj < 2; jj++) { const int c = g.c[jj + 1]; r.A7[jj] = a7[g.o + ro + c]; r.A7p[jj] = a7[g.op + ro + c]; }
+}
+
+__device__ __forceinline__ double lane_xor(double x, int m) {
+  const int idx = (__lane_id() ^ m) << 2;
+  const int lo = __builtin_amdgcn_ds_bpermute(idx, __double2loint(x)), hi = __builtin_amdgcn_ds_bpermute(idx, __double2hiint(x));
+  return __hiloint2double(hi, lo);
+}
+#define RR_XOR(x, m) (ZW ? lane_xor(x, m) : __shfl_xor(x, m, 64))
+
+}
+
+template <bool REAL, int AW, int AR, bool NORM = false, bool ZW = false>
 __global__ __launch_bounds__(256, 1) void k_residual_restrict(LevView F, LevView C, double *__restrict__ dst, Sides ph, double *__restrict__ zero, int gx, int gy,
                                                              double *__restrict__ partial = nullptr, double *__restrict__ dup = nullptr) {
-  __shared__ double red_ss[4];
-  double ss = 0.0;
+  __shared__ double red_ss[8];
+  static_assert(!(ZW && NORM), "the closing residual of solve_p streams its slots");
+  __shared__ double park[ZW ? 9 * 256 : 1];
+  const double *parked = park + threadIdx.y * 64 + threadIdx.x;
+  double ss = 0.0, sl = 0.0;
   int bx, by;
   if ((gy & 7) == 0) { const int xcd = blockIdx.x & 7, local = blockIdx.x >> 3; by = xcd * (gy >> 3) + local / gx; bx = local - (local / gx) * gx; }
   else { by = blockIdx.x / gx; bx = blockIdx.x - by * gx; }
@@ -67,7 +86,7 @@
   int j2 = 1 + bx * 32 + (threadIdx.x & 31);
   const int i2 = 1 + by * blockDim.y + threadIdx.y;
   if (i2 > C.nx) {
-    if (NORM) { if ((threadIdx.x & 63) == 0) red_ss[threadIdx.y] = 0.0; __syncthreads(); if (threadIdx.x == 0 && threadIdx.y == 0) partial[blockIdx.x] = red_ss[0] + red_ss[1] + red_ss[2] + red_ss[3]; }
+    if (NORM) { if ((threadIdx.x & 63) == 0) { red_ss[threadIdx.y] = 0.0; red_ss[4 + threadIdx.y] = 0.0; } __syncthreads(); }
     return;
   }
   const bool live = j2 <= C.ny;
@@ -93,6 +112,34 @@
       e[jj][4] = a8[g.o + c]; e[jj][5] = F.p[g.om + jm]; e[jj][6] = a8[g.op + jp]; e[jj][7] = F.p[g.op + jp];
     }
   }
+  double hh[6], hv[6], hz[6];
+  double m4[3], d4[3], r4[3], m7[2], d7[2], r7[2], m7p[2], d7p[2], r7p[2];
+  const double *__restrict__ cffw = F.cffw, *__restrict__ csw = F.csw;
+  RowR S1;
+  if (ZW) {
+    RowR Sn;
+    load_s(S1, F, g, 0);
+    load_s(Sn, F, g, (long long)(nz - 1) * RS);
+    const long long q2 = (long long)(2 * i2 - 1 + half) * RS, qf = half ? q2 + RS : q2 - RS;
+#pragma unroll
+    for (int jj = 0; jj < 2; jj++) {
+      hh[4 + jj] = F.h2[qf + g.c[jj + 1]]; hv[4 + jj] = F.hi2[qf + g.c[jj + 1]]; hz[4 + jj] = F.ze2[qf + g.c[jj + 1]];
+    }
+#pragma unroll
+    for (int q = 0; q < 4; q++) { hh[q] = F.h2[q2 + g.c[q]]; hv[q] = F.hi2[q2 + g.c[q]]; hz[q] = F.ze2[q2 + g.c[q]]; }
+#pragma unroll
+    for (int q = 0; q < 3; q++) { m4[q] = F.m4[q2 + g.c[q + 1]]; d4[q] = F.d4[q2 + g.c[q + 1]]; r4[q] = RCP_REF(d4[q]); }
+#pragma unroll
+    for (int jj = 0; jj < 2; jj++) {
+      m7[jj] = F.m7[q2 + g.c[jj + 1]]; d7[jj] = F.d7[q2 + g.c[jj + 1]]; r7[jj] = RCP_REF(d7[jj]);
+      m7p[jj] = F.m7[q2 + RS + g.c[jj + 1]]; d7p[jj] = F.d7[q2 + RS + g.c[jj + 1]]; r7p[jj] = RCP_REF(d7p[jj]);
+    }
+    double *mine = park + threadIdx.y * 64 + threadIdx.x;
+#pragma unroll
+    for (int q = 0; q < 3; q++) mine[q * 256] = Sn.A4[q];
+#pragma unroll
+    for (int jj = 0; jj < 2; jj++) { mine[(3 + jj) * 256] = Sn.A7[jj]; mine[(5 + jj) * 256] = Sn.A7p[jj]; mine[(7 + jj) * 256] = dlast[jj]; }
+  }
   constexpr int NWB = 3 + AW, NRB = 1 + AR;
   constexpr int U = (NWB % NRB == 0) ? NWB : NWB * NRB;
   static_assert(U <= 12, "unroll");
@@ -100,16 +147,16 @@
   RowR R[NRB];
 #pragma unroll
   for (int q = 0; q < AW + 2; q++) load_w(W[q], F, g, (long long)(q + 1 <= nz ? q : nz - 1) * RS);
-  load_r(R[NRB - 1], F, g, 0);
-#pragma unroll
-  for (int q = 0; q < AR - 1; q++) load_r(R[q], F, g, (long long)(q + 2 <= nz ? q + 1 : nz - 1) * RS);
+  load_r<ZW>(R[NRB - 1], F, g, 0);
+#pragma unroll
+  for (int q = 0; q < AR - 1; q++) load_r<ZW>(R[q], F, g, (long long)(q + 2 <= nz ? q + 1 : nz - 1) * RS);
   double z = 0.0;
   const long long oc = (long long)i2 * C.plane + jpos(C, j2);
 
 #define RR_LOADS(k, Wn, Rn)                                                                                                 \
     load_w(Wn, F, g, (long long)((k) + 1 + AW <= nz ? (k) + AW : nz - 1) * RS);                                              \
-    load_r(Rn, F, g, (long long)((k) + AR <= nz ? (k) + AR - 1 : nz - 1) * RS);
-#define RR_CELL_IN(Wm, W0, Wp, R0)                                                                                          \
+    load_r<ZW>(Rn, F, g, (long long)((k) + AR <= nz ? (k) + AR - 1 : nz - 1) * RS);
+#define RR_CELL_IN(Wm, W0, Wp, R0, S4, S7, S7P)                                                                                        \
       const double pc_m = Wm.P[jj + 1], pc_0 = W0.P[jj + 1], pc_p = Wp.P[jj + 1];                                            \
       const double pjm_m = Wm.P[jj], pjm_0 = W0.P[jj], pjm_p = Wp.P[jj];                                                     \
       const double pjp_m = Wm.P[jj + 2], pjp_0 = W0.P[jj + 2], pjp_p = Wp.P[jj + 2];                                         \
@@ -118,14 +165,14 @@
       const double zy_m = Wm.ZY4[jj + 1], zy_p = Wp.ZY4[jj + 1], zx_m = Wm.ZX[jj], zx_p = Wp.ZX[jj];                         \
       const double zyjm = W0.ZY4[jj], zyjp = W0.ZY4[jj + 2];                                                                \
       const double zxim = R0.ZXm[jj], zxip = R0.ZXp[jj];                                                                    \
-      const double a4o = R0.A4[jj], a4jp = R0.A4[jj + 1], a7o = R0.A7[jj], a7ip = R0.A7p[jj];                                \
+      const double a4o = S4[jj], a4jp = S4[jj + 1], a7o = S7[jj], a7ip = S7P[jj];                                            \
       const double a2_0 = W0.A2[jj], a2_p = Wp.A2[jj];                                                                      \
       const double c3 = qrt * (zy_p + zyjm), c3m = qrt * (zyjp + zy_m), c5 = -qrt * (zy_m + zyjm), c5m = -qrt * (zyjp + zy_p); \
       const double c6 = qrt * (zx_p + zxim), c6m = qrt * (zxip + zx_m), c8 = -qrt * (zx_m + zxim), c8m = -qrt * (zxip + zx_p); \
       (void)pc_m; (void)pjm_m; (void)pjp_m; (void)pim_m; (void)pip_m; (void)c3m; (void)c5; (void)c6m; (void)c8; (void)a2_0;
 #define RR_SUM(k, r)                                                                                                        \
-    if (NORM && live) ss = ss + (r[0] * r[0] + r[1] * r[1]);                                                                \
-    const double rA_B = __shfl_xor(r[0], 32, 64), rB_B = __shfl_xor(r[1], 32, 64);                                          \
+    if (NORM && live) { dd_add(ss, sl, r[0] * r[0]); dd_add(ss, sl, r[1] * r[1]); }                                         \
+    const double rA_B = RR_XOR(r[0], 32), rB_B = RR_XOR(r[1], 32);                                                          \
     if ((k) & 1) z = r[0] + rA_B + r[1] + rB_B;                                                                             \
     else {                                                                                                                  \
       z = z + r[0] + rA_B + r[1] + rB_B;                                                                                    \
@@ -145,30 +192,57 @@
                       - c6 * pim_p - c6m * pip_m - a7o * pim_0 - a7ip * pip_0                                                \
                       - c8 * pim_m - c8m * pip_p;                                                                            \
       }
-#define RR_LAST(rr, R0)                                                                                                     \
+#define RR_LAST(rr, R0, DL)                                                                                                 \
       {                                                                                                                     \
-        rr = R0.B[jj] - dlast[jj] * pc_0 - a2_0 * pc_m - c3m * pjp_m - a4o * pjm_0 - a4jp * pjp_0                           \
+        rr = R0.B[jj] - (DL) * pc_0 - a2_0 * pc_m - c3m * pjp_m - a4o * pjm_0 - a4jp * pjp_0                           \
                       - c5 * pjm_m - c6m * pip_m - a7o * pim_0 - a7ip * pip_0 - c8 * pim_m;                                  \
       }
+#define RR_ZW_ROW(kk, zo, zm, zp)                                                                                           \
+    {                                                                                                                       \
+      const int kz_ = (kk);                                                     \
+      _Pragma("unroll") for (int q = 0; q < 4; q++) zo[q] = ZW_GEN(kz_, q);                                                  \
+      _Pragma("unroll") for (int jj = 0; jj < 2; jj++) {                                                                     \
+        double zf_;                                                                                                         \
+        zf_ = ZW_GEN(kz_, 4 + jj);                                                                                                       \
+        const double zx_ = lane_xor(zo[jj + 1], 32);                                                                        \
+        zm[jj] = half ? zx_ : zf_; zp[jj] = half ? zf_ : zx_;                                                               \
+      }                                                                                                                     \
+    }
+#define RR_SLOTS(k)                                                                                                         \
+    double s4[3], s7[2], s7p[2];                                                                                            \
+    if (!ZW) ;                                                                                                              \
+    else if ((k) < nz) {                                                                                                    \
+      double zlo[4], zlm[2], zlp[2], zhi[4], zhm[2], zhp[2];                                                                \
+      RR_ZW_ROW(k, zlo, zlm, zlp)                                                                                           \
+      RR_ZW_ROW((k) + 1, zhi, zhm, zhp)                                                                                     \
+      _Pragma("unroll") for (int q = 0; q < 3; q++) s4[q] = DIVC(qrt * (zhi[q + 1] - zlo[q + 1] + zhi[q] - zlo[q]) * m4[q], d4[q], r4[q]); \
+      _Pragma("unroll") for (int jj = 0; jj < 2; jj++) {                                                                     \
+        s7[jj] = DIVC(qrt * (zhi[jj + 1] - zlo[jj + 1] + zhm[jj] - zlm[jj]) * m7[jj], d7[jj], r7[jj]);                       \
+        s7p[jj] = DIVC(qrt * (zhp[jj] - zlp[jj] + zhi[jj + 1] - zlo[jj + 1]) * m7p[jj], d7p[jj], r7p[jj]);                   \
+      }                                                                                                                     \
+    } else { _Pragma("unroll") for (int q = 0; q < 3; q++) s4[q] = parked[q * 256];                                          \
+             _Pragma("unroll") for (int jj = 0; jj < 2; jj++) { s7[jj] = parked[(3 + jj) * 256]; s7p[jj] = parked[(5 + jj) * 256]; } }
 #define RR_STEP(k, Wm, W0, Wp, Wn, R0, Rn)                                                                                  \
   {                                                                                                                         \
     RR_LOADS(k, Wn, Rn)                                                                                                     \
+    RR_SLOTS(k)                                                                                                             \
     double r[2];                                                                                                            \
     _Pragma("unroll") for (int jj = 0; jj < 2; jj++) {                                                                     \
-      RR_CELL_IN(Wm, W0, Wp, R0)                                                                                            \
+      RR_CELL_IN(Wm, W0, Wp, R0, (ZW ? s4 : R0.A4), (ZW ? s7 : R0.A7), (ZW ? s7p : R0.A7p))                                      \
       double rr;                                                                                                            \
       if ((k) < nz) RR_GENERAL(rr, R0)                                                                                       \
-      else RR_LAST(rr, R0)                                                                                                  \
+      else RR_LAST(rr, R0, ZW ? parked[(7 + jj) * 256] : dlast[jj])                                                         \
       r[jj] = rr;                                                                                                           \
     }                                                                                                                       \
     RR_SUM(k, r)                                                                                                            \
   }
   {
     RR_LOADS(1, W[AW + 2], R[AR - 1])
+    const RowR &R1 = ZW ? S1 : R[NRB - 1];
     double r[2];
 #pragma unroll
     for (int jj = 0; jj < 2; jj++) {
-      RR_CELL_IN(W[0], W[0], W[1], R[NRB - 1])
+      RR_CELL_IN(W[0], W[0], W[1], R[NRB - 1], R1.A4, R1.A7, R1.A7p)
       double rr = R[NRB - 1].B[jj] - dedge[jj] * pc_0 - a2_p * pc_p - c3 * pjm_p - a4o * pjm_0 - a4jp * pjp_0
                                    - c5m * pjp_p - c6 * pim_p - a7o * pim_0 - a7ip * pip_0 - c8m * pip_p;
       if (REAL) rr = rr - e[jj][0] * e[jj][1] - e[jj][2] * e[jj][3] - e[jj][4] * e[jj][5] - e[jj][6] * e[jj][7];
@@ -186,20 +260,26 @@
     if (k + q <= nz) RR_STEP(k + q, W[q % NWB], W[(q + 1) % NWB], W[(q + 2) % NWB], W[(q + 2 + AW) % NWB], R[q % NRB], R[(q + AR) % NRB])
   }
 #undef RR_STEP
+#undef RR_SLOTS
+#undef RR_ZW_ROW
 #undef RR_LOADS
   if (NORM) {
 #pragma unroll
-    for (int off = 32; off > 0; off >>= 1) ss += __shfl_xor(ss, off, 64);
-    if ((threadIdx.x & 63) == 0) red_ss[threadIdx.y] = ss;
+    for (int off = 32; off > 0; off >>= 1) { const double oh = __shfl_xor(ss, off, 64), ol = __shfl_xor(sl, off, 64); dd_merge(ss, sl, oh, ol); }
+    if ((threadIdx.x & 63) == 0) { red_ss[threadIdx.y] = ss; red_ss[4 + threadIdx.y] = sl; }
     __syncthreads();
-    if (threadIdx.x == 0 && threadIdx.y == 0) partial[blockIdx.x] = red_ss[0] + red_ss[1] + red_ss[2] + red_ss[3];
+    if (threadIdx.x == 0 && threadIdx.y == 0) {
+      for (int w = 1; w < 4; w++) dd_merge(ss, sl, red_ss[w], red_ss[4 + w]);
+      partial[blockIdx.x] = ss; partial[gridDim.x + blockIdx.x] = sl;
+    }
   }
 }
 
 template <bool REAL, int S, bool NORM = false>
 __global__ __launch_bounds__(64) void k_residual_restrict_flat(LevView F, LevView C, double *__restrict__ dst, Sides ph, double *__restrict__ zero, int gx,
                                                               double *__restrict__ partial = nullptr, double *__restrict__ dup = nullptr) {
-  double ss = 0.0;
+  constexpr bool ZW = false;
+  double ss = 0.0, sl = 0.0;
   const int nz = F.nz, nks = (nz + S - 1) / S, ng = gx * C.nx;
   int grp, ks;
   if ((ng & 7) == 0) { const int xcd = blockIdx.x & 7, local = blockIdx.x >> 3; ks = local % nks; grp = xcd * (ng >> 3) + local / nks; }
@@ -254,14 +334,14 @@
       double rv[2];
 #pragma unroll
       for (int jj = 0; jj < 2; jj++) {
-        RR_CELL_IN(W[r], W[r + 1], W[r + 2], R[r])
+        RR_CELL_IN(W[r], W[r + 1], W[r + 2], R[r], R[r].A4, R[r].A7, R[r].A7p)
         double rr;
         if (r == 0 && kr == 1) {
           rr = R[r].B[jj] - dedge[jj] * pc_0 - a2_p * pc_p - c3 * pjm_p - a4o * pjm_0 - a4jp * pjp_0
                           - c5m * pjp_p - c6 * pim_p - a7o * pim_0 - a7ip * pip_0 - c8m * pip_p;
           if (REAL) rr = rr - e[jj][0] * e[jj][1] - e[jj][2] * e[jj][3] - e[jj][4] * e[jj][5] - e[jj][6] * e[jj][7];
         } else if (kr < nz) RR_GENERAL(rr, R[r])
-        else RR_LAST(rr, R[r])
+        else RR_LAST(rr, R[r], dlast[jj])
         rv[jj] = rr;
       }
       RR_SUM(kr, rv)
@@ -269,11 +349,12 @@
   }
   if (NORM) {
 #pragma unroll
-    for (int off = 32; off > 0; off >>= 1) ss += __shfl_xor(ss, off, 64);
-    if (threadIdx.x == 0) partial[blockIdx.x] = ss;
+    for (int off = 32; off > 0; off >>= 1) { const double oh = __shfl_xor(ss, off, 64), ol = __shfl_xor(sl, off, 64); dd_merge(ss, sl, oh, ol); }
+    if (threadIdx.x == 0) { partial[blockIdx.x] = ss; partial[gridDim.x + blockIdx.x] = sl; }
   }
 }
 #undef RR_SUM
+#undef RR_XOR
 #undef RR_CELL_IN
 #undef RR_GENERAL
 #undef RR_LAST
@@ -307,14 +388,17 @@
   const int by = 4, gx = (C->ny + 31) / 32, gy = (C->nx + by - 1) / by;
   dim3 blk(WAVE, by), grd(gx * gy);
   const int deep = sw.resrest_ahead;
-#define RRW(REALV, AWV, ARV, NV) hipLaunchKernelGGL((k_residual_restrict<REALV, AWV, ARV, NV>), grd, blk, 0, st, *F, *C, dst, ph, zero, gx, gy, partial, dup)
-#define RRW2(AWV, ARV) { if (partial) { if (real) RRW(true, AWV, ARV, true); else RRW(false, AWV, ARV, true); } else { if (real) RRW(true, AWV, ARV, false); else RRW(false, AWV, ARV, false); } }
+  const bool zw = !sw.resrest_no_zw && !partial && F->m4 && F->d4 && F->m7 && F->d7 && F->h2 && F->hi2 && F->ze2 && F->cffw && F->csw;
+#define RRW(REALV, AWV, ARV, NV, ZV) hipLaunchKernelGGL((k_residual_restrict<REALV, AWV, ARV, NV, ZV>), grd, blk, 0, st, *F, *C, dst, ph, zero, gx, gy, partial, dup)
+#define RRW3(AWV, ARV, ZV) { if (partial) { if (real) RRW(true, AWV, ARV, true, ZV); else RRW(false, AWV, ARV, true, ZV); } else { if (real) RRW(true, AWV, ARV, false, ZV); else RRW(false, AWV, ARV, false, ZV); } }
+#define RRW2(AWV, ARV) RRW3(AWV, ARV, false)
   switch (deep) {
     case 12: RRW2(1, 2) break;
     case 21: RRW2(2, 1) break;
-    default: RRW2(1, 1) break;
+    default: if (zw) { if (real) RRW(true, 1, 1, false, true); else RRW(false, 1, 1, false, true); } else RRW2(1, 1) break;
   }
 #undef RRW2
+#undef RRW3
 #undef RRW
   return mgx_launched();
 }
diff --git a/mgroms_amd/csrc/mgx_switches.cpp b/mgroms_amd/csrc/mgx_switches.cpp
--- a/mgroms_amd/csrc/mgx_switches.cpp
+++ b/mgroms_amd/csrc/mgx_switches.cpp
@@ -36,6 +36,7 @@
   {"MGX_RESREST_FLAT_MAX",       &Switches::resrest_flat_max,      ATOLL,     256LL * 256 * 64, "fine cells up to which the fused residual + restriction takes its flat form (no walk up the column); same bits"},
   {"MGX_RESREST_FLAT_S",         &Switches::resrest_flat_s,        ATOI,      0,                ">= 4: four fine rows per wave in the flat form instead of two; same bits"},
   {"MGX_RESREST_AHEAD",          &Switches::resrest_ahead,         ATOI,      11,               "10 * AW + AR, the look-ahead of the walking form: 12 and 21 are instantiated beside 11; same bits"},
+  {"MGX_RESREST_NO_ZW",          &Switches::resrest_no_zw,         SET_TRUE,  0,                "the walking form of a cycle's down leg streams slots 4 and 7 instead of generating their interior rows from the depth formula (look-ahead 11, no norm: the others always stream); same bits"},
   {"MGX_P2P_MAXBLK",             &Switches::p2p_maxblk,            ATOI,      128,              "block cap of the halo push kernel (its grid must stay resident beside a neighbour's smoother); same bits"},
   {"MGX_P2P_IPT",                &Switches::p2p_ipt,               ATOI,      1,                "test hook: at least that many items per thread in the halo push kernel; same bits"},
   {"MGX_MODEL_KR",               &Switches::model_kr,              ATOI,      0,                "> 0 (A/B and test hook): runs of exactly that many rows in the flux kernels and correct_uvw; same bits"},
diff --git a/mgroms_amd/csrc/mgx_switches.h b/mgroms_amd/csrc/mgx_switches.h
--- a/mgroms_amd/csrc/mgx_switches.h
+++ b/mgroms_amd/csrc/mgx_switches.h
@@ -9,7 +9,7 @@
   bool rbseq_d0_kernel, rbseq_d0_mid, no_rbseq_walk_apply, rbseq_window_no_xmap;
   int rbw_prio;
   int c2f_kc, c2f_nt;
-  bool no_resrest;
+  bool no_resrest, resrest_no_zw;
   long long resrest_min, resrest_flat_max;
   int resrest_flat_s, resrest_ahead;
   int p2p_maxblk, p2p_ipt, model_kr;
```

Result: faster. 532.4 V-cycles/s (x number of 512x512x64 blocks when N>1: weak scaling) (median of 6 runs) (+1.6%).
